# yanconglin/ICP-Flow

Measured on AMD Instinct MI355X. Metric: cluster-pair ICP registrations/sec, higher is better.
Workload: dtype f32

## Files before the change

icp_flow_amd/_lib.py:

```python
import contextlib
import ctypes
import os
import threading

import torch

_HERE = os.path.dirname(os.path.abspath(__file__))
LIB_PATH = os.environ.get("ICPFLOW_HIP_LIB") or os.path.join(_HERE, "libicpflow_hip.so")

STOP_REFERENCE = 0
STOP_PER_PAIR = 1

if not os.path.exists(LIB_PATH):
    raise ImportError(
        f"{LIB_PATH} not found: build it with `python icp_flow_amd/build.py` "
        "(hipcc --offload-arch=gfx950).  icp_flow_amd has no CPU fallback.")

_L = ctypes.CDLL(LIB_PATH)

_f = ctypes.c_float
_d = ctypes.c_double
_i = ctypes.c_int
_p = ctypes.c_void_p
_sz = ctypes.c_size_t
# ... 2 lines not shown
    "icpflow_version": (_i, []),
    "icpflow_last_error": (ctypes.c_char_p, []),
    "icpflow_workspace_bytes": (_sz, [_i, _i, _i, _i, _i]),
    "icpflow_hist_vote": (_i, [_p, _p, _i, _i, _i, _f, _f, _f, _f, _f, _f, _i, _i, _i, _p, _p]),
    "icpflow_hist_peaks": (_i, [_p, _i, _i, _i, _i, _i, _i, _p, _p, _p, _sz, _p]),
    "icpflow_nn_batch": (_i, [_p, _p, _i, _i, _i, _i, _i, _p, _p, _i, _p, _p, _p]),
    "icpflow_transform_points": (_i, [_p, _p, _i, _i, _p, _p]),
    "icpflow_count_valid": (_i, [_p, _i, _i, _p, _p]),
    "icpflow_build_info": (ctypes.c_char_p, []),
    "icpflow_estimate_init_pose": (_i, [_p, _p, _i, _i, _p, _i, _p, _i, _p, _i, _f, _p, _p, _sz, _p, _p]),
    "icpflow_icp": (_i, [_p, _p, _p, _i, _i, _d, _i, _d, _i, _p, _p, _p, _p, _p, _p, _sz, _p, _p]),
    "icpflow_apply_icp": (_i, [_p, _p, _p, _i, _i, _d, _i, _d, _i, _p, _p, _p, _sz, _p, _p]),
    "icpflow_hist_icp": (_i, [_p, _p, _i, _i, _p, _i, _p, _i, _p, _i, _f, _d, _i, _d, _i, _p, _p, _p, _sz, _p, _p]),
    "icpflow_hist_icp_many": (_i, [_i, _p, _p, _p, _i, _p, _i, _p, _i, _p, _i, _f, _d, _i, _d, _i, _p, _p, _p, _p, _p, _p]),
    "icpflow_match_eval": (_i, [_p, _p, _p, _i, _i, _d, _p, _p, _p, _p, _p, _p, _p, _sz, _p, _p]),
    "icpflow_hist_icp_eval": (_i, [_p, _p, _i, _i, _p, _i, _p, _i, _p, _i, _f, _d, _i, _d, _i, _p, _p, _p, _p, _p, _p, _p,
                                   _p, _p, _sz, _p, _p]),
    "icpflow_gather_pad": (_i, [_p, _p, _i, _i, _p, _p]),
    "icpflow_gather_segments": (_i, [_p, _p, _p, _p, _i, _i, _p, _p]),
    "icpflow_assoc_assign": (_i, [_p, _p, _p, _i, _p, _i, _i, _f, _f, _f, _f, _p, _i, _p, _p, _p, _p, _p]),
    "icpflow_assoc_collect": (_i, [_p, _p, _p, _p, _i, _p, _p, _p, _p, _i, _p, _p, _i, _i, _i, _p, _p, _p, _p]),
    "icpflow_register_stage": (_i, [_p, _p, _p, _p, _sz, _p, _p]),
    "icpflow_associate_frame": (_i, [_p, _p, _p, _p, _p, _f, _f, _f, _f, _p, _i, _p, _p, _p, _p, _i, _p, _p, _p, _sz, _p, _p]),
    "icpflow_register_stage_begin": (_i, [_p, _p, _p, _p, _sz, _p, _p, _p]),
    "icpflow_register_stage_finish": (_i, [_p, _p, _p, _p, _sz, _p, _p, _p]),
    "icpflow_associate_frame_begun": (_i, [_p, _p, _p, _p, _p, _f, _f, _f, _f, _p, _i, _p, _p, _p, _p, _i, _p, _p, _p, _sz, _p, _p, _p]),
    "icpflow_track_frame": (_i, [_p, _p, _i, _p, _p, _i, _p, _p, _p, _p, _p, _p, _p, _p, _p, _sz, _p, _p, _p]),
    "icpflow_selftest_randperm": (_i, [_p, ctypes.c_int64, _i, _p]),
    "icpflow_cluster_stats": (_i, [_p, _p, _p, _p, _p, _i, _p, _p, _p]),
    "icpflow_cluster_table_workspace_bytes": (_sz, [_i, _i]),
    "icpflow_cluster_table": (_i, [_p, _p, _i, _p, _p, _i, _p, _p, _sz, _p]),
    "icpflow_cluster_table_pair_workspace_bytes": (_sz, [_i, _i, _i]),
    "icpflow_cluster_table_pair": (_i, [_p, _p, _i, _p, _p, _p, _p, _p, _i, _p, _p, _p, _i, _p, _sz, _p]),
    "icpflow_flow_rigid": (_i, [_p, _p, _i, _p, _p, _i, _p, _p, _p, _sz, _p]),
    "icpflow_flow_rigid_rows": (_i, [_p, _p, _i, _p, _i, _p, _i, _p, _p, _p]),
    "icpflow_dbscan_workspace_bytes": (_sz, [_i]),
    "icpflow_dbscan": (_i, [_p, _i, _p, _i, _d, _i, _p, _p, _p, _p, _sz, _p]),
    "icpflow_hdbscan_mst_workspace_bytes": (_sz, [_i]),
    "icpflow_hdbscan_mst": (_i, [_p, _i, _p, _i, _i, _d, _p, _p, _p, _p, _p, _p, _p, _sz, _p]),
    "icpflow_hdbscan_labels": (_i, [_p, _p, _p, _i, _i, _p]),
    "icpflow_ego_default_params": (_i, [_p]),
    "icpflow_ego_state_bytes": (_sz, [_p]),
    "icpflow_ego_create": (_i, [_p, _p, _sz, _p, ctypes.POINTER(_p)]),
    "icpflow_ego_destroy": (_i, [_p]),
    "icpflow_ego_reset": (_i, [_p, _p]),
    "icpflow_ego_register_frame": (_i, [_p, _p, _i, _p, _p]),
    "icpflow_ego_poses": (_i, [_p, _p, _i, ctypes.POINTER(_i)]),
    "icpflow_ego_frame_info": (_i, [_p, _p]),
    "icpflow_ego_downsample": (_i, [_p, _p, _i, _p, _p, _p, _p]),
    "icpflow_ego_register_step": (_i, [_p, _p, _i, _p, _d, _p, _p]),
    "icpflow_ego_map_add": (_i, [_p, _p, _i, _p, _p]),
    "icpflow_ego_map_export": (_i, [_p, _p, _p, _p, _i, _p, _p]),
    "icpflow_selftest_vote_quotient": (_i, [_p, _i, _f, _f, _p, _p, _p]),
    "icpflow_selftest_kabsch": (_i, [_p, _p, _i, _i, _p, _p, _p, _p]),
    "icpflow_profile_create": (_i, [_i, ctypes.POINTER(_p)]),
    "icpflow_profile_collect": (_i, [_p, ctypes.POINTER(_d), ctypes.POINTER(_i)]),
    "icpflow_profile_destroy": (_i, [_p]),
}
for _name, (_res, _args) in SIGNATURES.items():
    _fn = getattr(_L, _name)
    _fn.restype = _res
    _fn.argtypes = _args

VERSION = int(_L.icpflow_version())
BUILD_INFO = _L.icpflow_build_info().decode()


def call(name, *args):
    rc = getattr(_L, name)(*args)
    if rc != 0:
        msg = _L.icpflow_last_error()
        raise RuntimeError(f"{name} failed (code {rc}): {msg.decode() if msg else ''}")


SEARCH_AUTO, SEARCH_SCAN, SEARCH_GRID, SEARCH_SWEEP = 0, 1, 2, 3
ARITH_FP64, ARITH_FP32_REFERENCE = 0, 1
OPT_FLAGS = {"no_sorted_vote": 1 << 0, "no_side_stream": 1 << 1, "no_eval_sweep": 1 << 2, "no_check_sweep": 1 << 3,
             "no_score_sweep": 1 << 4, "no_score_prune": 1 << 5, "no_teams": 1 << 6, "no_speculative": 1 << 7,
             "no_adaptive_windows": 1 << 8, "no_persistent": 1 << 9, "no_helpers": 1 << 10,
             "teams_half_gpu": 1 << 11, "no_shared_scans": 1 << 12,
             "no_stage_overlap": 1 << 13, "no_vote_list": 1 << 14, "no_check_reuse": 1 << 15, "no_score_prebound": 1 << 16,
             "two_launch": 1 << 17,
             "no_dir_keys": 1 << 18}


class Options(ctypes.Structure):
    _fields_ = [("struct_size", _sz), ("icp_search", _i), ("icp_arith", _i), ("flags", ctypes.c_uint),
                ("profile", _p), ("d_vote_bins_u32", _p), ("d_icp_init_R", _p), ("d_icp_init_T", _p),
                ("d_icp_history", _p), ("icp_allow_reflection", _i), ("icp_estimate_scale", _i),
                ("d_icp_scale", _p), ("d_icp_init_s", _p), ("d_pair_active", _p)]


class Tables(ctypes.Structure):
    _fields_ = [("d_points_src", _p), ("d_order_src", _p), ("d_table_src", _p), ("d_points_dst", _p), ("d_order_dst", _p),
                ("d_table_dst", _p), ("S", _i), ("D", _i), ("label_stride", _i)]


class Stage(ctypes.Structure):
    _fields_ = [("d_seg", _p), ("d_perm", _p), ("d_si", _p), ("d_di", _p), ("d_clouds", _p), ("d_result", _p), ("K", _i), ("N", _i)]


class Registration(ctypes.Structure):
    _fields_ = [("d_edges_x", _p), ("d_edges_y", _p), ("d_edges_z", _p), ("len_x", _i), ("len_y", _i), ("len_z", _i),
                ("decode_shift", _f), ("thres_dist", _d), ("relative_rmse_thr", _d), ("max_iterations", _i), ("stop_mode", _i)]


class Mt19937(ctypes.Structure):
    _fields_ = [("state", ctypes.c_uint32 * 624), ("index", ctypes.c_int32)]

    @staticmethod
    def from_torch(generator=None):
        raw = (generator if generator is not None else torch.default_generator).get_state().numpy()
        if raw.size < 24 + 8 * 624:
            raise RuntimeError("unexpected layout of torch.Generator.get_state()")
        left = int(raw[8:12].view("<i4")[0])
        nxt = int(raw[16:24].view("<u8")[0])
        mt = Mt19937()
        ctypes.memmove(mt.state, raw[24:24 + 8 * 624].view("<u8").astype("<u4").tobytes(), 4 * 624)
        mt.index = 624 if left == 1 else nxt
        return mt

    def to_torch(self, generator=None):
        import numpy as np
        g = generator if generator is not None else torch.default_generator
        raw = g.get_state().numpy().copy()
        raw[24:24 + 8 * 624] = np.frombuffer(bytes(self.state), dtype="<u4").astype("<u8").view(np.uint8)
        idx = int(self.index)
        raw[8:12] = np.array([1 if idx >= 624 else 625 - idx], "<i4").view(np.uint8)
        raw[16:24] = np.array([idx], "<u8").view(np.uint8)
        g.set_state(torch.from_numpy(raw))


class FrameParams(ctypes.Structure):
    _fields_ = [("struct_size", _sz), ("seed", ctypes.c_uint64), ("generator", _p), ("max_points", _i), ("min_cluster_size", _i),
                ("translation_frame", _f), ("thres_box", _f), ("thres_iou", _f), ("rot_limit_deg", _f), ("thres_error", _f),
                ("tight_padding", _i), ("superset_width", _i)]


class EgoParams(ctypes.Structure):
    _fields_ = [("struct_size", _sz), ("max_range", _d), ("min_range", _d), ("voxel_size", _d), ("min_motion_th", _d),
                ("initial_threshold", _d), ("convergence", _d), ("max_points_per_voxel", _i), ("max_iterations", _i),
                ("max_points", _i), ("map_capacity", _i)]

    @staticmethod
    def defaults(**over):
        p = EgoParams()
        call("icpflow_ego_default_params", ctypes.byref(p))
        for k, v in over.items():
            if not hasattr(p, k):
                raise TypeError(f"icpflow_ego_params_t has no field {k!r}")
            setattr(p, k, v)
        return p


class Profile:

    def __init__(self, capacity):
        self._h = _p()
        call("icpflow_profile_create", int(capacity), ctypes.byref(self._h))

    def collect(self):
        ms, n = _d(0.0), _i(0)
        call("icpflow_profile_collect", self._h, ctypes.byref(ms), ctypes.byref(n))
        return float(ms.value), int(n.value)

    def close(self):
        if self._h:
            _L.icpflow_profile_destroy(self._h)
            self._h = _p()

    __del__ = close


_tls = threading.local()


def _env_default_flags():
    f = 0
    for name, bit in OPT_FLAGS.items():
        if os.environ.get("ICPFLOW_" + name.upper(), "0") not in ("0", ""):
            f |= bit
    return f


_DEFAULT_FLAGS = _env_default_flags()


def _current():
    return getattr(_tls, "stack", None) or [dict(search=0, arith=0, flags=_DEFAULT_FLAGS, profile=None, vote_bins=None,
                                                 icp_init=None, icp_history=None, icp_allow_reflection=False,
                                                 icp_scale=None, pair_active=None)]


@contextlib.contextmanager
def options(search=None, arith=None, profile=None, vote_bins=None, icp_init=None, icp_history=None,
            icp_allow_reflection=None, icp_scale=None, pair_active=None, **switches):
    cur = dict(_current()[-1])
    cur.update(vote_bins=None, icp_init=None, icp_history=None, icp_scale=None, pair_active=None)
    if search is not None:
        cur["search"] = {"auto": 0, "scan": 1, "grid": 2, "sweep": 3}.get(search, search)
    if arith is not None:
        cur["arith"] = {"fp64": 0, "fp32_reference": 1}.get(arith, arith)
    if profile is not None:
        cur["profile"] = profile
    if vote_bins is not None:
        cur["vote_bins"] = vote_bins
    if icp_init is not None:
        cur["icp_init"] = icp_init
    if icp_history is not None:
        cur["icp_history"] = icp_history
    if icp_allow_reflection is not None:
        cur["icp_allow_reflection"] = bool(icp_allow_reflection)
    if icp_scale is not None:
        cur["icp_scale"] = icp_scale
    if pair_active is not None:
        cur["pair_active"] = pair_active
    for k, v in switches.items():
        cur["flags"] = (cur["flags"] | OPT_FLAGS[k]) if v else (cur["flags"] & ~OPT_FLAGS[k])
    stack = getattr(_tls, "stack", None)
    if stack is None:
        stack = _tls.stack = []
    stack.append(cur)
    try:
        yield
    finally:
        stack.pop()


def opt():
    cur = _current()[-1]
    if (cur["search"] == 0 and cur["arith"] == 0 and cur["flags"] == 0 and cur["profile"] is None
            and cur["vote_bins"] is None and cur["icp_init"] is None and cur["icp_history"] is None
            and not cur["icp_allow_reflection"] and cur["icp_scale"] is None and cur.get("pair_active") is None):
        return None
    dp = lambda t: ctypes.c_void_p(t.data_ptr()) if t is not None else None
    o = Options(int(os.environ.get("ICPFLOW_OPTIONS_SIZE", ctypes.sizeof(Options))), int(cur["search"]), int(cur["arith"]), int(cur["flags"]),
                cur["profile"]._h if cur["profile"] is not None else None, dp(cur["vote_bins"]),
                dp(cur["icp_init"][0] if cur["icp_init"] is not None else None),
                dp(cur["icp_init"][1] if cur["icp_init"] is not None else None), dp(cur["icp_history"]),
                1 if cur["icp_allow_reflection"] else 0, 1 if cur["icp_scale"] is not None else 0, dp(cur["icp_scale"]),
                dp(cur["icp_init"][2] if cur["icp_init"] is not None and len(cur["icp_init"]) > 2 else None),
                dp(cur.get("pair_active")))
    _tls.last = o
    return ctypes.cast(ctypes.pointer(o), _p)


def workspace_bytes(B, N, lens=(0, 0, 0)):
    return int(_L.icpflow_workspace_bytes(int(B), int(N), int(lens[0]), int(lens[1]), int(lens[2])))


def require_gpu(*tensors):
    for t in tensors:
        if t is None:
            continue
        if not isinstance(t, torch.Tensor) or not t.is_cuda:
            raise RuntimeError("icp_flow_amd: input must be a GPU (HIP) tensor -- there is no CPU path "
                               "(the reference refuses CPU tensors too, hist_cuda/cpp/hist.cpp:22)")


def cloud(t, name="cloud"):
    require_gpu(t)
    if t.dim() != 3 or t.shape[2] != 4:
        raise RuntimeError(f"{name}: expected shape [B,N,4] (x,y,z,flag), got {tuple(t.shape)}")
    if t.dtype != torch.float32:
        raise RuntimeError(f"{name}: expected float32, got {t.dtype}")
    return t.contiguous()


def ptr(t):
    return ctypes.c_void_p(t.data_ptr()) if t is not None else None


_raw_stream = getattr(torch._C, "_cuda_getCurrentRawStream", None)


def stream_handle(device):
    if _raw_stream is not None:
        idx = device.index if isinstance(device, torch.device) else None
        if idx is None:
            idx = torch.cuda.current_device()
        return int(_raw_stream(idx))
    return int(torch.cuda.current_stream(device).cuda_stream)


def stream(device):
    return ctypes.c_void_p(stream_handle(device))


_ws_cache = {}


def workspace(device, nbytes):
    key = (device.type, device.index, stream_handle(device))
    buf = _ws_cache.get(key)
    if buf is None or buf.numel() < nbytes:
        buf = torch.empty(max(int(nbytes), 1 << 20), dtype=torch.uint8, device=device)
        _ws_cache[key] = buf
    return buf


def workspaces(device, sizes):
# ... 20 lines not shown
```

icp_flow_amd/csrc/api.hip:

```cpp
#include <stdarg.h>
#include <stdio.h>
#include <stdlib.h>
#include <string.h>

#include "kernels.hpp"
#include "posefuse.hpp"
#include "kabsch.hpp"

using namespace icpflow;

namespace {

thread_local char g_err[512] = "";

int fail(int code, const char *fmt, ...)
{
    va_list ap;
    va_start(ap, fmt);
    vsnprintf(g_err, sizeof(g_err), fmt, ap);
    va_end(ap);
    return code;
}

int hipfail(hipError_t e, const char *what)
// ... 60 lines not shown
    int arith = ICPFLOW_ARITH_FP64;
    unsigned flags = 0u;
    LaunchProfile *profile = nullptr;
    uint32_t *voteBins = nullptr;
    const float *initR = nullptr, *initT = nullptr;
    float *history = nullptr;
    bool allowReflection = false;
    bool estimateScale = false;
    float *scaleOut = nullptr;
    const float *initS = nullptr;
    const uint8_t *pairActive = nullptr;
    bool on(unsigned offFlag) const { return (flags & offFlag) == 0u; }
    IcpOpts icp(float *scratch) const
    {
        IcpOpts o;
        o.fp32Scratch = scratch;
        o.ctrlCleared = true;
        o.arith = arith;
        o.teams = on(ICPFLOW_OPT_NO_TEAMS);
        o.speculative = on(ICPFLOW_OPT_NO_SPECULATIVE);
        o.adaptiveWindows = on(ICPFLOW_OPT_NO_ADAPTIVE_WINDOWS);
        o.persistent = on(ICPFLOW_OPT_NO_PERSISTENT);
        o.helpers = on(ICPFLOW_OPT_NO_HELPERS);
        o.teamsHalfGpu = (flags & ICPFLOW_OPT_TEAMS_HALF_GPU) != 0u;
        o.sharedScans = on(ICPFLOW_OPT_NO_SHARED_SCANS);
        o.twoLaunch = (flags & ICPFLOW_OPT_TWO_LAUNCH) != 0u;
        o.pairActive = pairActive;
        o.profile = profile;
        return o;
    }
};

#ifndef ICPFLOW_SCORE_SWEEP_MIN_N
#define ICPFLOW_SCORE_SWEEP_MIN_N 2048
#endif
constexpr int kScoreSweepMinN = ICPFLOW_SCORE_SWEEP_MIN_N;
constexpr int kMaxSortN = 16384;
inline bool eval_by_sweep(int B, int N, const Opts &o)
{
    if (N > kMaxSortN || !o.on(ICPFLOW_OPT_NO_EVAL_SWEEP)) return false;
    return N > kScoreSweepMinN || (N >= 1024 && (long long)B * N >= (1LL << 18));
}
#ifndef ICPFLOW_SCORE_SWEEP_MIN_N_SORTED
#define ICPFLOW_SCORE_SWEEP_MIN_N_SORTED 512
#endif
constexpr int kScoreSweepMinNSorted = ICPFLOW_SCORE_SWEEP_MIN_N_SORTED;
inline bool score_by_sweep(int N, bool sortedAnyway, const Opts &o)
{
    const int minN = (sortedAnyway && o.on(ICPFLOW_OPT_NO_SCORE_PRUNE)) ? kScoreSweepMinNSorted : kScoreSweepMinN;
    return N > minN && N <= kMaxSortN && o.on(ICPFLOW_OPT_NO_SCORE_SWEEP);
}
constexpr size_t kAlign = 256;
size_t up(size_t n) { return (n + kAlign - 1) / kAlign * kAlign; }

struct Workspace {
    int32_t *lenA = nullptr, *lenC = nullptr;
    uint8_t *swap = nullptr;
    uint32_t *bins = nullptr, *volA = nullptr, *volB = nullptr;
    float *peakVotes = nullptr;
    int64_t *peakIdx = nullptr;
    float *cand = nullptr;
    double *scoreAccum = nullptr;
    double *partial = nullptr;
    float *Tinit = nullptr, *M = nullptr;
    IcpState *state = nullptr;
    IcpCtrl *ctrl = nullptr;
    float *helpState = nullptr;
    double *helpOut = nullptr;
    GridScratch grid{};
    float *history = nullptr;
    float *zsortA = nullptr, *zsortC = nullptr;
    float *zckey = nullptr;
    int32_t *voteWork = nullptr;
    size_t voteWorkCap = 0;
    int32_t *pairTab = nullptr;
    int32_t *pairOrder = nullptr;
    float *pairBox = nullptr;
    float *voteKey = nullptr;
    int *zcidx = nullptr;
    IcpTeam team{};
    int32_t *icpSplit = nullptr;
    bool initSumValid = false;
    int *ticketScratch = nullptr;
    size_t accumBytes = 0;
    size_t bytes = 0;
    static bool shareScratch(int B, int N) { return N >= 2048 && (size_t)B * 12 * kSweepShareSlots * 256 * 4 <= ((size_t)64 << 20); }

    Workspace(void *base, int B, int N, size_t L)
    {
        size_t off = 0;
        auto take = [&](size_t n) {
            void *p = base ? (void *)((char *)base + off) : nullptr;
            off += up(n);
            return p;
        };
        const size_t b = (size_t)B;
        lenA = (int32_t *)take(b * 4);
        lenC = (int32_t *)take(b * 4);
        swap = (uint8_t *)take(b);
        bins = (uint32_t *)take(b * L * 4);
        volA = (uint32_t *)take(b * L * 4);
        volB = (uint32_t *)take(b * L * 4);
        peakVotes = (float *)take(b * kTopK * 4);
        peakIdx = (int64_t *)take(b * kTopK * 8);
        cand = (float *)take(b * kCand * 3 * 4);
        {
            size_t qb = (size_t)(scan_qblocks(N, B) > sweep_qblocks(N) ? scan_qblocks(N, B) : sweep_qblocks(N));
            if ((size_t)score_qblocks(N) > qb) qb = (size_t)score_qblocks(N);
            partial = (double *)take(b * 12 * qb * kPartial * 8);
            scoreAccum = (double *)take(b * 12 * 8);
            ticketScratch = (int *)take(256);
            if (shareScratch(B, N)) grid.shareCount = (int *)take(b * 12 * kSweepShareSlots * 4);
            accumBytes = up(b * 12 * 8) + up(256) + (shareScratch(B, N) ? up(b * 12 * kSweepShareSlots * 4) : 0);
        }
        Tinit = (float *)take(b * 16 * 4);
        M = (float *)take(b * 16 * 4);
        state = (IcpState *)take(b * sizeof(IcpState));
        ctrl = (IcpCtrl *)take(icp_ctrl_bytes(B));
        helpState = (float *)take(b * 32 * 4);
        helpOut = (double *)take((size_t)kHelpMaxWG * kHelpOutStride * 8);
        grid.H = grid_buckets(N);
        grid.origin = (float *)take(b * 4 * 4);
        grid.start = (int32_t *)take(b * ((size_t)grid.H + 1) * 4);
        grid.cursor = (int32_t *)take(b * (size_t)grid.H * 4);
        grid.pts = (float *)take(b * (size_t)N * 16);
        grid.sortX = (float *)take(b * (size_t)N * 16);
        grid.sortYsoa = (float *)take(b * 3 * (size_t)((N + 15) / 16 * 16) * 4 + 256);
        grid.sortXsoa = (float *)take(b * 3 * (size_t)((N + 15) / 16 * 16) * 4 + 256);
        zsortA = (float *)take(b * (size_t)N * 16);
        zsortC = (float *)take(b * (size_t)N * 16);
        voteKey = (float *)take(b * 8 * 4);
        voteWorkCap = vote_work_capacity(B, N);
        if (voteWorkCap != 0) { voteWork = (int32_t *)take(voteWorkCap * 4); pairOrder = (int32_t *)take(b * 4); }
        if (N > kChunkSortMinN) {
            const size_t cs = b * 2 * (size_t)chunk_sort_length(N) * 4;
            grid.ckey = (float *)take(cs);
            grid.cidx = (int *)take(cs);
            zckey = (float *)take(cs);
            zcidx = (int *)take(cs);
            pairBox = (float *)take(b * kPairBoxStride * 4);
        }
        grid.axis = (int32_t *)take(b * 4);
        grid.scoreList = (int *)take(b * 12 * 4);
        if (N <= kMaxSortN) {
            grid.occHdr = (float *)take(b * 2 * 8 * 4);
            grid.occBits = (uint32_t *)take(b * 2 * (size_t)kOccRings * kOccWords * 4);
        }
        if (shareScratch(B, N)) {
            grid.shareBest = (float *)take(b * 12 * kSweepShareSlots * 256 * 4);
            if (B <= 32767 && N <= 255 * 256) pairTab = (int32_t *)take(b * 4 * 4);
        }
        history = (float *)take(b * (size_t)kHistIters * kHistStride * 4);
        team.maxWG = 1024;
        team.wgPair = (int32_t *)take((size_t)team.maxWG * 4);
        team.wgRank = (int32_t *)take((size_t)team.maxWG * 4);
        team.teamSize = (int32_t *)take(b * 4);
        team.next = (int32_t *)take(b * 4);
        team.arrived = (unsigned int *)take(b * 4);
        team.mom = (double *)take((b < 256 ? b : 256) * 2 * (size_t)kMaxTeam * kTeamStride * 8);
        icpSplit = (int32_t *)take((b + 64) * 4);
        bytes = off;
    }
};

const GridScratch *search_scratch(Workspace &w, int N, const Opts &o)
{
    int mode = o.search;
    if (o.arith == ICPFLOW_ARITH_FP32_REFERENCE) mode = 1;
    if (mode == 0) mode = (N >= 64 && N <= kMaxSortN) ? 3 : 1;
    if (mode == 3 && N > kMaxSortN) mode = 1;
    if (mode == 1) return nullptr;
    w.grid.mode = mode;
    w.grid.dirKeys = o.on(ICPFLOW_OPT_NO_DIR_KEYS) ? 1 : 0;
    return &w.grid;
}

int parse_options(const char *fn, const icpflow_options_t *opt, Opts &o)
{
    if (opt == nullptr) return 0;
    if (opt->struct_size != sizeof(icpflow_options_t))
        return fail(ICPFLOW_E_ARG, "%s: options struct_size %zu, this library expects %zu", fn, opt->struct_size,
                    sizeof(icpflow_options_t));
    if (opt->icp_search < 0 || opt->icp_search > 3)
        return fail(ICPFLOW_E_ARG, "%s: options.icp_search must be 0..3 (got %d)", fn, opt->icp_search);
    if (opt->icp_arith != ICPFLOW_ARITH_FP64 && opt->icp_arith != ICPFLOW_ARITH_FP32_REFERENCE)
        return fail(ICPFLOW_E_ARG, "%s: options.icp_arith must be 0 or 1 (got %d)", fn, opt->icp_arith);
    if (opt->flags >> 19) return fail(ICPFLOW_E_ARG, "%s: unknown option flags 0x%x", fn, opt->flags);
    o.search = opt->icp_search;
    o.arith = opt->icp_arith;
    o.flags = opt->flags;
    o.profile = reinterpret_cast<LaunchProfile *>(opt->profile);
    o.voteBins = opt->d_vote_bins_u32;
    if ((opt->d_icp_init_R == nullptr) != (opt->d_icp_init_T == nullptr))
        return fail(ICPFLOW_E_ARG, "%s: options.d_icp_init_R and d_icp_init_T come together", fn);
    o.initR = opt->d_icp_init_R;
    o.initT = opt->d_icp_init_T;
    o.history = opt->d_icp_history;
    o.allowReflection = opt->icp_allow_reflection != 0;
    o.estimateScale = opt->icp_estimate_scale != 0;
    o.scaleOut = opt->d_icp_scale;
    o.initS = opt->d_icp_init_s;
    o.pairActive = opt->d_pair_active;
    if (o.initS != nullptr && o.initR == nullptr)
        return fail(ICPFLOW_E_ARG, "%s: options.d_icp_init_s comes with d_icp_init_R / d_icp_init_T", fn);
    return 0;
}

int check_pair_active(const char *fn, const Opts &o, bool fused, int maxIter, int stopMode)
{
    if (o.pairActive == nullptr) return 0;
    if (!fused) return fail(ICPFLOW_E_ARG, "%s: options.d_pair_active is honoured by icpflow_hist_icp / icpflow_hist_icp_eval only", fn);
    if (stopMode != ICPFLOW_STOP_REFERENCE || maxIter < 2 || maxIter > kHistIters || !o.on(ICPFLOW_OPT_NO_SPECULATIVE) ||
        o.arith != ICPFLOW_ARITH_FP64)
        return fail(ICPFLOW_E_ARG, "%s: options.d_pair_active needs the single-launch reference stop (2 <= max_iterations <= %d, "
                                   "fp64 arithmetic, speculation on)", fn, kHistIters);
    return 0;
}

int check_arith(const char *fn, const Opts &o, int maxIter, int stopMode)
{
    if (o.arith != ICPFLOW_ARITH_FP32_REFERENCE) return 0;
    if (stopMode != ICPFLOW_STOP_REFERENCE)
        return fail(ICPFLOW_E_ARG, "%s: ICPFLOW_ARITH_FP32_REFERENCE implements the reference's batch-global stop only", fn);
    if (maxIter > kHistIters)
        return fail(ICPFLOW_E_LIMIT, "%s: ICPFLOW_ARITH_FP32_REFERENCE keeps a per-iteration history: max_iterations <= %d",
                    fn, kHistIters);
    return 0;
}

int check_ws(void *ws, size_t have, size_t need)
{
    if (ws == nullptr || have < need)
        return fail(ICPFLOW_E_WORKSPACE, "workspace too small: have %zu bytes, need %zu", have, need);
    if (((uintptr_t)ws & 15) != 0) return fail(ICPFLOW_E_WORKSPACE, "workspace must be 16-byte aligned");
    return 0;
}

int check_batch(const char *fn, int B, int N)
{
    if (B <= 0 || N <= 0) return fail(ICPFLOW_E_ARG, "%s: B (%d) and N (%d) must be positive", fn, B, N);
    if ((long long)B * N > (1ll << 30)) return fail(ICPFLOW_E_LIMIT, "%s: B*N exceeds 2^30 rows", fn);
    return 0;
}

int check_hist_dims(const char *fn, int lx, int ly, int lz)
{
    if (lx <= 0 || ly <= 0 || lz <= 0)
        return fail(ICPFLOW_E_ARG, "%s: histogram lengths must be positive (%d,%d,%d)", fn, lx, ly, lz);
    if ((long long)lx * ly * lz > (1ll << 28)) return fail(ICPFLOW_E_LIMIT, "%s: histogram too large", fn);
    return 0;
}

struct SideStream {
    hipStream_t stream = nullptr;
    hipEvent_t fork = nullptr, join = nullptr;
    int device = -1;
    bool ok = false;
    void destroy()
    {
        if (stream) (void)hipStreamDestroy(stream);
        if (fork) (void)hipEventDestroy(fork);
        if (join) (void)hipEventDestroy(join);
        stream = nullptr; fork = join = nullptr; ok = false;
    }
    void create()
    {
        ok = hipGetDevice(&device) == hipSuccess &&
             hipStreamCreateWithFlags(&stream, hipStreamNonBlocking) == hipSuccess &&
             hipEventCreateWithFlags(&fork, hipEventDisableTiming) == hipSuccess &&
             hipEventCreateWithFlags(&join, hipEventDisableTiming) == hipSuccess;
    }
};

SideStream &side_stream(hipStream_t caller)
{
    constexpr int kSlots = 6;
    struct Slot { SideStream s; hipStream_t caller = nullptr; bool used = false; };
    static thread_local Slot slots[kSlots];
    static thread_local int next = 0;
    static thread_local SideStream none;
    int dev = -1;
    if (hipGetDevice(&dev) != hipSuccess) { none.ok = false; return none; }
    for (int k = 0; k < kSlots; ++k)
        if (slots[k].used && slots[k].caller == caller && slots[k].s.device == dev) return slots[k].s;
    Slot &sl = slots[next];
    next = (next + 1) % kSlots;
    if (!sl.used || sl.s.device != dev) {
        sl.s.destroy();
        sl.s = SideStream{};
        sl.s.create();
    }
    sl.used = true;
    sl.caller = caller;
    return sl.s;
}

struct JoinGuard {
    hipStream_t s = nullptr;
    hipEvent_t join = nullptr;
    ~JoinGuard() { if (join != nullptr) (void)hipStreamWaitEvent(s, join, 0); }
    void joined() { join = nullptr; }
};

int run_icp_and_select(const float *src, const float *dst, Workspace &w, const uint8_t *swap,
                       const float *init, int B, int N, double thres, int maxIter, double relThr,
                       int stopMode, int invertSwapped, float *Tout, int32_t *iters, const Opts &o, hipStream_t s,
                       bool teamPlanned = false, int part = 0, int32_t *pending = nullptr, bool initSumValid = false)
{
    const GridScratch *search = search_scratch(w, N, o);
    const bool sweepCheck = search != nullptr && search->mode == 3 && o.on(ICPFLOW_OPT_NO_CHECK_SWEEP);
    bool historyPending = false;
    IcpOpts io = o.icp(w.grid.sortX);
    io.help = icp_help_carve(w.ctrl, B, w.helpState, w.helpOut);
    io.splitScratch = w.icpSplit;
    io.teamPlanned = teamPlanned;
    if (sweepCheck && o.arith == ICPFLOW_ARITH_FP64) io.historyPending = &historyPending;
    const bool splittable = sweepCheck && o.arith == ICPFLOW_ARITH_FP64 && stopMode == ICPFLOW_STOP_REFERENCE && w.history != nullptr &&
                            o.on(ICPFLOW_OPT_NO_SPECULATIVE) && maxIter > 1 && maxIter <= kHistIters;
    if (part == 1) {
        *pending = 0;
        if (!splittable) return 0;
        if (icp_teams_wanted(&w.team, io, search, B, N, maxIter, stopMode, w.history)) return 0;
        io.pairActive = nullptr;
    }
    if (part == 2 && pending != nullptr && *pending != 0) {
        historyPending = true;
        if (o.pairActive != nullptr) ICPFLOW_TRY(launch_icp_retally(w.ctrl, w.history, o.pairActive, B, maxIter, relThr, s));
    } else {
        ICPFLOW_TRY(launch_icp(src, dst, w.lenA, w.lenC, swap, init, B, N, thres, maxIter, relThr, stopMode,
                               w.state, w.ctrl, search, w.history, &w.team, io, s));
        if (part == 1) {
            if (!historyPending) return fail(ICPFLOW_E_ARG, "icpflow_register_stage_begin: the ICP launch kept no history");
            *pending = 1;
            return 0;
        }
    }
    if (sweepCheck) {
        PoseSource ps{w.state, w.ctrl, historyPending ? w.history : nullptr, init, B, maxIter};
        const double *initSum = (initSumValid && search->presorted && o.on(ICPFLOW_OPT_NO_CHECK_REUSE)) ? w.scoreAccum : nullptr;
        ICPFLOW_TRY(launch_sweep_check(search, src, dst, w.lenA, w.lenC, swap, B, N, init, nullptr, w.partial, s, &ps, o.pairActive,
                                       initSum));
        ICPFLOW_TRY(launch_select(w.partial, sweep_qblocks(N), w.lenA, w.lenC, swap, init, nullptr, B, invertSwapped,
                                  Tout, s, &ps, iters, initSum, o.pairActive));
        return 0;
    }
    ICPFLOW_TRY(launch_compose(w.state, init, B, w.M, s, w.ctrl, iters));
    {
        ICPFLOW_TRY(launch_scan_check(src, dst, w.lenA, w.lenC, swap, B, N, init, w.M, w.partial, s));
        ICPFLOW_TRY(launch_select(w.partial, scan_qblocks(N, B), w.lenA, w.lenC, swap, init, w.M, B,
                                  invertSwapped, Tout, s));
    }
    return 0;
}

int run_init_pose(const float *src, const float *dst, Workspace &w, const uint8_t *swap, int B,
                  int N, const float *ex, int lx, const float *ey, int ly, const float *ez, int lz,
                  float shift, float *Tout, const Opts &o, hipStream_t s, hipEvent_t joinBefore = nullptr,
                  const PairCountFuse *countFuse = nullptr, bool sideBusy = false)
{
    const int lens[3] = {lx, ly, lz};
    if (N <= kMaxSortN && o.on(ICPFLOW_OPT_NO_SORTED_VOTE)) {
        bool planned = false;
        ICPFLOW_TRY(launch_hist_vote_sorted(dst, src, w.lenC, w.lenA, B, N, lens, ex, ey, ez, swap, w.zsortC,
                                            w.zsortA, w.bins, w.zckey, w.zcidx, w.voteKey, s, countFuse, sideBusy,
                                            w.grid.pairBox, o.on(ICPFLOW_OPT_NO_VOTE_LIST) ? w.voteWork : nullptr, w.voteWorkCap,
                                            w.pairOrder, &planned));
        if (planned) w.grid.pairOrder = w.pairOrder;
    } else
        ICPFLOW_TRY(launch_hist_vote(dst, src, B, N, N, nullptr, nullptr, lens, ex, ey, ez, swap, w.bins, s));
    if (o.voteBins != nullptr)
        ICPFLOW_TRY(hipMemcpyAsync(o.voteBins, w.bins, (size_t)B * lx * ly * lz * sizeof(uint32_t),
                                   hipMemcpyDeviceToDevice, s));
    if (w.pairTab != nullptr && B <= 700 && N <= kMaxSortN && o.on(ICPFLOW_OPT_NO_SORTED_VOTE)) {
        ICPFLOW_TRY(launch_sweep_pair_table(w.lenA, w.lenC, swap, w.grid.pairOrder, B, N, w.pairTab, s));
        w.grid.pairTab = w.pairTab;
    }
    PeakDecode dec;
    dec.ex = ex; dec.ey = ey; dec.ez = ez; dec.shift = shift; dec.cand = w.cand;
    ICPFLOW_TRY(launch_hist_peaks_u32(w.bins, B, lx, ly, lz, kTopK, kNmsKernel, w.volA, w.volB,
                                      w.peakVotes, w.peakIdx, s, dec));
    if (score_by_sweep(N, joinBefore != nullptr || w.grid.presorted, o)) {
        if (joinBefore != nullptr) {
            ICPFLOW_TRY(hipStreamWaitEvent(s, joinBefore, 0));
        } else if (!w.grid.presorted) {
            ICPFLOW_TRY(launch_sort_clouds_soa(src, dst, w.lenA, w.lenC, swap, B, N, &w.grid, s));
            w.grid.presorted = 1;
            if (o.on(ICPFLOW_OPT_NO_SCORE_PRUNE) && o.on(ICPFLOW_OPT_NO_SCORE_PREBOUND)) {
                ICPFLOW_TRY(launch_occupancy(&w.grid, B, N, s));
                w.grid.occReady = 1;
            }
        }
        if (o.on(ICPFLOW_OPT_NO_SCORE_PRUNE))
            ICPFLOW_TRY(launch_sweep_score_pruned(&w.grid, w.lenA, w.lenC, swap, B, N, w.cand, w.partial, w.scoreAccum, s));
        else
            ICPFLOW_TRY(launch_sweep_score(&w.grid, w.lenA, w.lenC, swap, B, N, w.cand, w.partial, s));
        ICPFLOW_TRY(launch_score_pick(w.partial, sweep_qblocks(N), w.lenA, w.lenC, swap, w.cand, B, Tout, s, w.scoreAccum));
        w.initSumValid = true;
    } else if (o.on(ICPFLOW_OPT_NO_SCORE_PRUNE)) {
        ICPFLOW_TRY(launch_scan_score_pruned(src, dst, w.lenA, w.lenC, swap, B, N, w.cand, w.partial, w.scoreAccum, s, true));
        ICPFLOW_TRY(launch_score_pick(w.partial, score_qblocks(N), w.lenA, w.lenC, swap, w.cand, B, Tout, s));
    } else {
        ICPFLOW_TRY(launch_scan_score(src, dst, w.lenA, w.lenC, swap, B, N, w.cand, w.partial, s));
        ICPFLOW_TRY(launch_score_pick(w.partial, scan_qblocks(N, B), w.lenA, w.lenC, swap, w.cand, B, Tout, s));
    }
    return 0;
}

}

extern "C" {

int icpflow_version(void) { return ICPFLOW_VERSION; }

#ifndef ICPFLOW_SOURCE_HASH
#define ICPFLOW_SOURCE_HASH "unknown"
#endif
static const char g_build_info[] = "ICPFLOW_SOURCE_HASH=" ICPFLOW_SOURCE_HASH;
const char *icpflow_build_info(void) { return g_build_info + sizeof("ICPFLOW_SOURCE_HASH=") - 1; }

const char *icpflow_last_error(void) { return g_err; }

size_t icpflow_workspace_bytes(int B, int N, int Lx, int Ly, int Lz)
{
    if (B <= 0 || N <= 0) return 0;
    const size_t L = (size_t)(Lx > 0 ? Lx : 0) * (size_t)(Ly > 0 ? Ly : 0) * (size_t)(Lz > 0 ? Lz : 0);
    return Workspace(nullptr, B, N, L).bytes;
}

int icpflow_profile_create(int capacity, icpflow_profile_t **out)
{
    if (out == nullptr) return fail(ICPFLOW_E_ARG, "icpflow_profile_create: null pointer");
    if (capacity < 0 || capacity > (1 << 20)) return fail(ICPFLOW_E_ARG, "icpflow_profile_create: bad capacity %d", capacity);
    hipError_t e = hipSuccess;
    LaunchProfile *p = profile_create(capacity, &e);
    if (p == nullptr) return hipfail(e, "icpflow_profile_create");
    *out = reinterpret_cast<icpflow_profile_t *>(p);
    return 0;
}

int icpflow_profile_collect(icpflow_profile_t *profile, double *total_ms, int *launches)
{
    if (profile == nullptr) return fail(ICPFLOW_E_ARG, "icpflow_profile_collect: null recorder");
    ICPFLOW_TRY(profile_collect(reinterpret_cast<LaunchProfile *>(profile), total_ms, launches));
    return 0;
}

int icpflow_profile_destroy(icpflow_profile_t *profile)
{
    profile_destroy(reinterpret_cast<LaunchProfile *>(profile));
    return 0;
}

int icpflow_selftest_vote_quotient(const float *d_a, int n, float min_v, float max_v, float *d_fast,
                                   float *d_ieee, icpflow_stream_t stream)
{
    if (!d_a || !d_fast || !d_ieee) return fail(ICPFLOW_E_ARG, "icpflow_selftest_vote_quotient: null pointer");
    if (n <= 0) return fail(ICPFLOW_E_ARG, "icpflow_selftest_vote_quotient: n must be positive");
    ICPFLOW_TRY(launch_vote_quotient_probe(d_a, n, min_v, max_v, d_fast, d_ieee, (hipStream_t)stream));
    return 0;
}

int icpflow_selftest_kabsch(const double *d_H, const double *d_gsum, int n, int mode, double *d_R, double *d_lam,
                            int32_t *d_path, icpflow_stream_t stream)
{
    if (!d_H || !d_R || !d_lam || !d_path || (mode != 2 && !d_gsum))
        return fail(ICPFLOW_E_ARG, "icpflow_selftest_kabsch: null pointer");
    if (n <= 0 || n > (1 << 24)) return fail(ICPFLOW_E_ARG, "icpflow_selftest_kabsch: bad n %d", n);
    if (mode < 0 || mode > 2) return fail(ICPFLOW_E_ARG, "icpflow_selftest_kabsch: bad mode %d", mode);
    ICPFLOW_TRY(launch_kabsch_probe(d_H, d_gsum, n, mode, d_R, d_lam, d_path, (hipStream_t)stream));
    return 0;
}

int icpflow_hist_vote(const float *d_X, const float *d_Y, int B, int NX, int NY, float min_x,
                      float min_y, float min_z, float max_x, float max_y, float max_z, int len_x,
                      int len_y, int len_z, float *d_bins, icpflow_stream_t stream)
{
    if (!d_X || !d_Y || !d_bins) return fail(ICPFLOW_E_ARG, "icpflow_hist_vote: null pointer");
    if (int r = check_batch("icpflow_hist_vote", B, NX)) return r;
    if (int r = check_batch("icpflow_hist_vote", B, NY)) return r;
    if (int r = check_hist_dims("icpflow_hist_vote", len_x, len_y, len_z)) return r;
// ... 286 lines not shown
        return fail(ICPFLOW_E_WORKSPACE, "icpflow_cluster_table: workspace too small (%zu bytes, need %zu)", ws_bytes,
                    icpflow_cluster_table_workspace_bytes(M, Lmax));
    return 0;
}

size_t icpflow_cluster_table_pair_workspace_bytes(int MA, int MB, int Lmax)
{
    if (MA <= 0 || MB <= 0 || Lmax <= 0 || (long long)MA + MB > 0x7fffffffll) return 0;
    size_t bytes = 0;
    if (cluster_table_pair_workspace_bytes(MA, MB, Lmax, &bytes) != hipSuccess) return 0;
    return bytes;
}

int icpflow_cluster_table_pair(const float *d_points_a, const float *d_labels_a, int MA, int64_t *d_order_a, double *d_table_a,
                               int32_t *d_num_a, const float *d_points_b, const float *d_labels_b, int MB,
                               int64_t *d_order_b, double *d_table_b, int32_t *d_num_b, int Lmax, void *d_ws, size_t ws_bytes,
                               icpflow_stream_t stream)
{
    if (!d_points_a || !d_labels_a || !d_order_a || !d_table_a || !d_num_a || !d_points_b || !d_labels_b || !d_order_b ||
        !d_table_b || !d_num_b)
        return fail(ICPFLOW_E_ARG, "icpflow_cluster_table_pair: null pointer");
    if (MA <= 0 || MB <= 0) return fail(ICPFLOW_E_ARG, "icpflow_cluster_table_pair: MA, MB must be positive (got %d, %d)", MA, MB);
    if ((long long)MA + MB > 0x7fffffffll)
        return fail(ICPFLOW_E_LIMIT, "icpflow_cluster_table_pair: MA + MB must stay below 2^31 (got %d + %d)", MA, MB);
    if (Lmax <= 0 || Lmax > 4096) return fail(ICPFLOW_E_LIMIT, "icpflow_cluster_table_pair: 1 <= Lmax <= 4096 (got %d)", Lmax);
    if (!d_ws) return fail(ICPFLOW_E_WORKSPACE, "icpflow_cluster_table_pair: workspace is NULL");
    bool tooSmall = false;
    ICPFLOW_TRY(launch_cluster_table_pair(d_points_a, d_labels_a, MA, d_order_a, d_table_a, d_num_a, d_points_b, d_labels_b, MB,
                                          d_order_b, d_table_b, d_num_b, Lmax, d_ws, ws_bytes, &tooSmall, (hipStream_t)stream));
    if (tooSmall)
        return fail(ICPFLOW_E_WORKSPACE, "icpflow_cluster_table_pair: workspace too small (%zu bytes, need %zu)", ws_bytes,
                    icpflow_cluster_table_pair_workspace_bytes(MA, MB, Lmax));
    return 0;
}

int icpflow_flow_rigid_rows(const float *d_points, const float *d_labels, int N, const float *d_pair_rows, int pair_stride,
                            const float *d_T, int P, const float *d_pose, float *d_flow, icpflow_stream_t stream)
{
    if (!d_points || !d_labels || !d_pose || !d_flow) return fail(ICPFLOW_E_ARG, "icpflow_flow_rigid: null pointer");
    if (N <= 0) return fail(ICPFLOW_E_ARG, "icpflow_flow_rigid: N must be positive");
    if (P < 0 || P > (1 << 24)) return fail(ICPFLOW_E_LIMIT, "icpflow_flow_rigid: 0 <= P <= 2^24 pairs (got %d)", P);
    if (P > 0 && (!d_pair_rows || !d_T)) return fail(ICPFLOW_E_ARG, "icpflow_flow_rigid: null pair arrays");
    if (pair_stride < 1 || pair_stride > 1024)
        return fail(ICPFLOW_E_ARG, "icpflow_flow_rigid: pair_stride must be in 1 ... 1024 floats (got %d)", pair_stride);
    ICPFLOW_TRY(launch_flow_rigid(d_points, d_labels, N, d_pair_rows, pair_stride, d_T, P, d_pose, d_flow, (hipStream_t)stream));
    return 0;
}

int icpflow_flow_rigid(const float *d_points, const float *d_labels, int N, const float *d_pair_labels,
                       const float *d_T, int P, const float *d_pose, float *d_flow, void *d_ws, size_t ws_bytes,
                       icpflow_stream_t stream)
{
    (void)d_ws;
    (void)ws_bytes;
    return icpflow_flow_rigid_rows(d_points, d_labels, N, d_pair_labels, 1, d_T, P, d_pose, d_flow, stream);
}

int icpflow_count_valid(const float *d_pts, int B, int N, int32_t *d_len, icpflow_stream_t stream)
{
    if (!d_pts || !d_len) return fail(ICPFLOW_E_ARG, "icpflow_count_valid: null pointer");
    if (int r = check_batch("icpflow_count_valid", B, N)) return r;
    launch_count_valid(d_pts, B, N, d_len, (hipStream_t)stream);
    ICPFLOW_TRY(hipGetLastError());
    return 0;
}

int icpflow_estimate_init_pose(const float *d_src, const float *d_dst, int B, int N,
                               const float *d_edges_x, int len_x, const float *d_edges_y, int len_y,
                               const float *d_edges_z, int len_z, float decode_shift, float *d_T_out,
                               void *d_ws, size_t ws_bytes, icpflow_stream_t stream, const icpflow_options_t *opt)
{
    Opts o;
    if (int r = parse_options("icpflow_estimate_init_pose", opt, o)) return r;
    if (int r = check_pair_active("icpflow_estimate_init_pose", o, false, 0, 0)) return r;
    if (!d_src || !d_dst || !d_edges_x || !d_edges_y || !d_edges_z || !d_T_out)
        return fail(ICPFLOW_E_ARG, "icpflow_estimate_init_pose: null pointer");
    if (int r = check_batch("icpflow_estimate_init_pose", B, N)) return r;
    if (int r = check_hist_dims("icpflow_estimate_init_pose", len_x, len_y, len_z)) return r;
    const size_t L = (size_t)len_x * len_y * len_z;
    if (L < (size_t)kTopK) return fail(ICPFLOW_E_ARG, "icpflow_estimate_init_pose: fewer than 5 bins");
    Workspace w(d_ws, B, N, L);
    if (int r = check_ws(d_ws, ws_bytes, w.bytes)) return r;
    hipStream_t s = (hipStream_t)stream;
    launch_count_pair(d_src, d_dst, B, N, w.lenA, w.lenC, nullptr, s, w.scoreAccum, (size_t)B * 12 * sizeof(double));
    return run_init_pose(d_src, d_dst, w, nullptr, B, N, d_edges_x, len_x, d_edges_y, len_y, d_edges_z,
                         len_z, decode_shift, d_T_out, o, s);
}

int icpflow_icp(const float *d_X, const float *d_Y, const float *d_pre_pose, int B, int N, double thres,
                int max_iterations, double relative_rmse_thr, int stop_mode, float *d_R, float *d_T,
                float *d_rmse, int32_t *d_iters, int32_t *d_converged, void *d_ws, size_t ws_bytes,
                icpflow_stream_t stream, const icpflow_options_t *opt)
{
    Opts o;
    if (int r = parse_options("icpflow_icp", opt, o)) return r;
    if (int r = check_pair_active("icpflow_icp", o, false, 0, 0)) return r;
    if (int r = check_arith("icpflow_icp", o, max_iterations, stop_mode)) return r;
    if (!d_X || !d_Y) return fail(ICPFLOW_E_ARG, "icpflow_icp: null pointer");
    if (int r = check_batch("icpflow_icp", B, N)) return r;
    if (max_iterations <= 0 || max_iterations > kMaxIterCap)
        return fail(ICPFLOW_E_ARG, "icpflow_icp: max_iterations must be in 1..%d (got %d)", kMaxIterCap, max_iterations);
    if (stop_mode != ICPFLOW_STOP_REFERENCE && stop_mode != ICPFLOW_STOP_PER_PAIR)
        return fail(ICPFLOW_E_ARG, "icpflow_icp: unknown stop_mode %d", stop_mode);
    Workspace w(d_ws, B, N, 0);
    if (int r = check_ws(d_ws, ws_bytes, w.bytes)) return r;
    hipStream_t s = (hipStream_t)stream;
    IcpOpts io = o.icp(w.grid.sortX);
    io.help = icp_help_carve(w.ctrl, B, w.helpState, w.helpOut);
    io.splitScratch = w.icpSplit;
    io.initR = o.initR;
    io.initT = o.initT;
    io.allowReflection = o.allowReflection;
    io.estimateScale = o.estimateScale;
    io.initS = o.initS;
    if ((o.allowReflection || o.estimateScale) && o.arith != ICPFLOW_ARITH_FP64)
        return fail(ICPFLOW_E_ARG, "icpflow_icp: allow_reflection / estimate_scale are not built for ICPFLOW_ARITH_FP32_REFERENCE");
    if (o.history != nullptr &&
        !(stop_mode == ICPFLOW_STOP_REFERENCE && max_iterations > 1 && max_iterations <= kHistIters &&
          o.arith == ICPFLOW_ARITH_FP64 && io.speculative))
        return fail(ICPFLOW_E_ARG, "icpflow_icp: options.d_icp_history needs the single-launch reference stop mode "
                                   "(2 <= max_iterations <= %d, fp64 arithmetic)", kHistIters);
    if (o.initR != nullptr && o.arith != ICPFLOW_ARITH_FP64)
        return fail(ICPFLOW_E_ARG, "icpflow_icp: an initial transform is not built for ICPFLOW_ARITH_FP32_REFERENCE");
    Opts os = o;
    if ((o.estimateScale || o.initS != nullptr) && o.search == 0 && N < 64) os.search = 3;
    const GridScratch *search = search_scratch(w, N, os);
    if ((o.estimateScale || o.initS != nullptr) && (search == nullptr || search->mode != 3))
        return fail(ICPFLOW_E_ARG, "icpflow_icp: estimate_scale / an initial transform with a scale need the sorted-sweep "
                                   "search (the default up to N = %d)", kMaxSortN);
    launch_count_pair(d_X, d_Y, B, N, w.lenA, w.lenC, nullptr, s, w.ctrl, icp_ctrl_bytes(B));
    ICPFLOW_TRY(launch_icp(d_X, d_Y, w.lenA, w.lenC, nullptr, d_pre_pose, B, N, thres, max_iterations,
                           relative_rmse_thr, stop_mode, w.state, w.ctrl, search, w.history, &w.team,
                           io, s));
    if (o.history != nullptr)
        ICPFLOW_TRY(hipMemcpyAsync(o.history, w.history, (size_t)max_iterations * B * kHistStride * sizeof(float),
                                   hipMemcpyDeviceToDevice, s));
    ICPFLOW_TRY(launch_icp_export(w.state, w.ctrl, B, stop_mode, d_R, d_T, d_rmse, d_iters, d_converged, s, o.scaleOut));
    return 0;
}

int icpflow_apply_icp(const float *d_src, const float *d_dst, const float *d_init, int B, int N,
                      double thres_dist, int max_iterations, double relative_rmse_thr, int stop_mode,
                      float *d_T_out, int32_t *d_iters, void *d_ws, size_t ws_bytes,
                      icpflow_stream_t stream, const icpflow_options_t *opt)
{
    Opts o;
    if (int r = parse_options("icpflow_apply_icp", opt, o)) return r;
    if (int r = check_arith("icpflow_apply_icp", o, max_iterations, stop_mode)) return r;
    if (int r = check_pair_active("icpflow_apply_icp", o, false, max_iterations, stop_mode)) return r;
    if (!d_src || !d_dst || !d_init || !d_T_out) return fail(ICPFLOW_E_ARG, "icpflow_apply_icp: null pointer");
    if (int r = check_batch("icpflow_apply_icp", B, N)) return r;
    if (max_iterations <= 0 || max_iterations > kMaxIterCap)
        return fail(ICPFLOW_E_ARG, "icpflow_apply_icp: max_iterations must be in 1..%d", kMaxIterCap);
    if (stop_mode != ICPFLOW_STOP_REFERENCE && stop_mode != ICPFLOW_STOP_PER_PAIR)
        return fail(ICPFLOW_E_ARG, "icpflow_apply_icp: unknown stop_mode %d", stop_mode);
    Workspace w(d_ws, B, N, 0);
    if (int r = check_ws(d_ws, ws_bytes, w.bytes)) return r;
    hipStream_t s = (hipStream_t)stream;
    launch_count_pair(d_src, d_dst, B, N, w.lenA, w.lenC, nullptr, s, w.ctrl, icp_ctrl_bytes(B));
    ICPFLOW_TRY(hipMemcpyAsync(w.Tinit, d_init, (size_t)B * 16 * sizeof(float), hipMemcpyDeviceToDevice, s));
    return run_icp_and_select(d_src, d_dst, w, nullptr, w.Tinit, B, N, thres_dist, max_iterations,
                              relative_rmse_thr, stop_mode, 0, d_T_out, d_iters, o, s);
}

static int hist_icp_core(const float *d_src, const float *d_dst, int B, int N, const float *d_edges_x, int len_x,
                         const float *d_edges_y, int len_y, const float *d_edges_z, int len_z, float decode_shift,
                         double thres_dist, int max_iterations, double relative_rmse_thr, int stop_mode,
                         float *d_T_out, int32_t *d_iters, Workspace &w, const Opts &o, hipStream_t s,
                         int phase = 0, int32_t *carry = nullptr)
{
    if (phase == 2) {
        w.grid.presorted = carry[0];
        w.grid.shareCountClean = 1;
        int32_t pending = carry[2];
        return run_icp_and_select(d_src, d_dst, w, w.swap, w.Tinit, B, N, thres_dist, max_iterations,
                                  relative_rmse_thr, stop_mode, 1, d_T_out, d_iters, o, s, carry[1] != 0, 2, &pending, carry[3] != 0);
    }
    const bool countInSort = N <= kMaxSortN && N <= kChunkSortMinN && o.on(ICPFLOW_OPT_NO_SORTED_VOTE);
    if (!countInSort) {
        launch_count_pair(d_src, d_dst, B, N, w.lenA, w.lenC, w.swap, s, w.ctrl, icp_ctrl_bytes(B), w.scoreAccum,
                          w.accumBytes, w.pairBox);
        w.grid.pairBox = w.pairBox;
    }
    hipEvent_t join = nullptr;
    bool teamPlanned = false;
    JoinGuard guard;
    const GridScratch *search = search_scratch(w, N, o);
    SideStream *side = nullptr;
    if (search != nullptr && search->mode == 3 && N >= 64 && o.on(ICPFLOW_OPT_NO_SIDE_STREAM)) {
        side = &side_stream(s);
        if (!side->ok) side = nullptr;
    }
    if (side != nullptr) {
        ICPFLOW_TRY(hipEventRecord(side->fork, s));
        ICPFLOW_TRY(hipStreamWaitEvent(side->stream, side->fork, 0));
        hipError_t se = launch_sort_clouds_soa(d_src, d_dst, w.lenA, w.lenC, w.swap, B, N, &w.grid, side->stream,
                                               countInSort ? 2 : 0);
        if (se == hipSuccess && score_by_sweep(N, true, o) && o.on(ICPFLOW_OPT_NO_SCORE_PRUNE) && o.on(ICPFLOW_OPT_NO_SCORE_PREBOUND)) {
            se = launch_occupancy(&w.grid, B, N, side->stream);
            if (se == hipSuccess) w.grid.occReady = 1;
        }
        if (se == hipSuccess && !countInSort && phase != 1 &&
            icp_teams_wanted(&w.team, o.icp(w.grid.sortX), search, B, N, max_iterations, stop_mode, w.history)) {
            launch_icp_team_plan(&w.team, w.lenA, w.lenC, w.swap, B, N, o.icp(w.grid.sortX), side->stream);
            teamPlanned = true;
        }
        const hipError_t je = hipEventRecord(side->join, side->stream);
        if (je == hipSuccess) { guard.s = s; guard.join = side->join; }
        ICPFLOW_TRY(se);
        ICPFLOW_TRY(je);
        w.grid.presorted = 1;
        join = side->join;
    }
    PairCountFuse fuse{};
    if (countInSort) {
        fuse.swapOut = w.swap;
        fuse.zero0 = w.ctrl; fuse.bytes0 = icp_ctrl_bytes(B);
        fuse.zero1 = w.scoreAccum; fuse.bytes1 = w.accumBytes;
    }
    w.grid.shareCountClean = 1;
    w.grid.sweepTicket = w.ticketScratch;
    const bool sweepScore = score_by_sweep(N, join != nullptr, o);
    if (int r = run_init_pose(d_src, d_dst, w, w.swap, B, N, d_edges_x, len_x, d_edges_y, len_y, d_edges_z,
                              len_z, decode_shift, w.Tinit, o, s, sweepScore ? join : nullptr,
                              countInSort ? &fuse : nullptr, join != nullptr))
        return r;
    if (join != nullptr && !sweepScore) ICPFLOW_TRY(hipStreamWaitEvent(s, join, 0));
    guard.joined();
    if (phase == 1) {
        carry[0] = w.grid.presorted;
        carry[1] = teamPlanned ? 1 : 0;
        carry[3] = w.initSumValid ? 1 : 0;
        return run_icp_and_select(d_src, d_dst, w, w.swap, w.Tinit, B, N, thres_dist, max_iterations, relative_rmse_thr,
                                  stop_mode, 1, d_T_out, d_iters, o, s, teamPlanned, 1, &carry[2]);
    }
    return run_icp_and_select(d_src, d_dst, w, w.swap, w.Tinit, B, N, thres_dist, max_iterations,
                              relative_rmse_thr, stop_mode, 1, d_T_out, d_iters, o, s, teamPlanned, 0, nullptr, w.initSumValid);
}

int icpflow_hist_icp(const float *d_src, const float *d_dst, int B, int N, const float *d_edges_x,
                     int len_x, const float *d_edges_y, int len_y, const float *d_edges_z, int len_z,
                     float decode_shift, double thres_dist, int max_iterations, double relative_rmse_thr,
                     int stop_mode, float *d_T_out, int32_t *d_iters, void *d_ws, size_t ws_bytes,
                     icpflow_stream_t stream, const icpflow_options_t *opt)
{
    Opts o;
    if (int r = parse_options("icpflow_hist_icp", opt, o)) return r;
    if (int r = check_arith("icpflow_hist_icp", o, max_iterations, stop_mode)) return r;
    if (int r = check_pair_active("icpflow_hist_icp", o, true, max_iterations, stop_mode)) return r;
    if (!d_src || !d_dst || !d_edges_x || !d_edges_y || !d_edges_z || !d_T_out)
        return fail(ICPFLOW_E_ARG, "icpflow_hist_icp: null pointer");
    if (int r = check_batch("icpflow_hist_icp", B, N)) return r;
    if (int r = check_hist_dims("icpflow_hist_icp", len_x, len_y, len_z)) return r;
    if (max_iterations <= 0 || max_iterations > kMaxIterCap)
        return fail(ICPFLOW_E_ARG, "icpflow_hist_icp: max_iterations must be in 1..%d", kMaxIterCap);
    if (stop_mode != ICPFLOW_STOP_REFERENCE && stop_mode != ICPFLOW_STOP_PER_PAIR)
        return fail(ICPFLOW_E_ARG, "icpflow_hist_icp: unknown stop_mode %d", stop_mode);
    const size_t L = (size_t)len_x * len_y * len_z;
    if (L < (size_t)kTopK) return fail(ICPFLOW_E_ARG, "icpflow_hist_icp: fewer than 5 bins");
    Workspace w(d_ws, B, N, L);
    if (int r = check_ws(d_ws, ws_bytes, w.bytes)) return r;
    return hist_icp_core(d_src, d_dst, B, N, d_edges_x, len_x, d_edges_y, len_y, d_edges_z, len_z, decode_shift,
                         thres_dist, max_iterations, relative_rmse_thr, stop_mode, d_T_out, d_iters, w, o,
                         (hipStream_t)stream);
}

int icpflow_hist_icp_many(int K, const float *const *d_src, const float *const *d_dst, const int *B, int N,
                          const float *d_edges_x, int len_x, const float *d_edges_y, int len_y,
                          const float *d_edges_z, int len_z, float decode_shift, double thres_dist,
                          int max_iterations, double relative_rmse_thr, int stop_mode, float *const *d_T_out,
                          int32_t *const *d_iters, void *const *d_ws, const size_t *ws_bytes,
                          icpflow_stream_t stream, const icpflow_options_t *opt)
{
    if (K <= 0 || K > 64) return fail(ICPFLOW_E_ARG, "icpflow_hist_icp_many: K must be in 1..64 (got %d)", K);
    if (!d_src || !d_dst || !B || !d_T_out || !d_iters || !d_ws || !ws_bytes)
        return fail(ICPFLOW_E_ARG, "icpflow_hist_icp_many: null pointer");
    for (int k = 0; k < K; ++k)
        for (int j = 0; j < k; ++j)
            if (d_ws[k] == d_ws[j]) return fail(ICPFLOW_E_WORKSPACE, "icpflow_hist_icp_many: batches %d and %d share a workspace", j, k);
    hipStream_t s = (hipStream_t)stream;
    constexpr int kWorkers = 4;
    struct Pool {
        hipStream_t w[kWorkers] = {nullptr, nullptr, nullptr, nullptr};
        hipEvent_t fork = nullptr, join[kWorkers] = {nullptr, nullptr, nullptr, nullptr};
        int device = -1;
        bool ok = false;
    };
    static thread_local Pool pool;
    int dev = -1;
    ICPFLOW_TRY(hipGetDevice(&dev));
    if (!pool.ok || pool.device != dev) {
        pool = Pool{};
        pool.device = dev;
        ICPFLOW_TRY(hipEventCreateWithFlags(&pool.fork, hipEventDisableTiming));
        for (int k = 0; k < kWorkers; ++k) {
            ICPFLOW_TRY(hipStreamCreateWithFlags(&pool.w[k], hipStreamNonBlocking));
            ICPFLOW_TRY(hipEventCreateWithFlags(&pool.join[k], hipEventDisableTiming));
        }
        pool.ok = true;
    }
    const int used = K < kWorkers ? K : kWorkers;
    ICPFLOW_TRY(hipEventRecord(pool.fork, s));
    for (int k = 0; k < used; ++k) ICPFLOW_TRY(hipStreamWaitEvent(pool.w[k], pool.fork, 0));
    int rc = 0;
    for (int k = 0; k < K && rc == 0; ++k)
        rc = icpflow_hist_icp(d_src[k], d_dst[k], B[k], N, d_edges_x, len_x, d_edges_y, len_y, d_edges_z, len_z, decode_shift,
                              thres_dist, max_iterations, relative_rmse_thr, stop_mode, d_T_out[k], d_iters[k], d_ws[k],
                              ws_bytes[k], pool.w[k % kWorkers], opt);
    for (int k = 0; k < used; ++k) {
        const hipError_t e1 = hipEventRecord(pool.join[k], pool.w[k]);
        const hipError_t e2 = e1 == hipSuccess ? hipStreamWaitEvent(s, pool.join[k], 0) : e1;
        if (rc == 0 && e2 != hipSuccess) rc = hipfail(e2, "icpflow_hist_icp_many: join");
    }
    return rc;
}
// ... 126 lines not shown
```

icp_flow_amd/csrc/kernels.hpp:

```cpp
#pragma once
#include <hip/hip_runtime.h>
#include <atomic>
#include <stddef.h>
#include <stdint.h>

#include "../../include/icpflow_hip.h"

namespace icpflow {

constexpr int ICPFLOW_STOP_REFERENCE_ = ICPFLOW_STOP_REFERENCE;
constexpr int ICPFLOW_STOP_PER_PAIR_ = ICPFLOW_STOP_PER_PAIR;

constexpr int kPartial = 8;
constexpr int kMaxIterCap = 1024;
constexpr int kCand = 6;
constexpr int kTopK = 5;
constexpr int kNmsKernel = 11;

struct IcpState {
    float R[9];
    float T[3];
    float rmse;
    int active;
    int iters;
// ... 41 lines not shown
struct IcpTeam {
    int32_t *wgPair;
    int32_t *wgRank;
    int32_t *teamSize;
    int32_t *next;
    unsigned int *arrived;
    double *mom;
    int maxWG;
};

inline size_t icp_ctrl_bytes(int B)
{
    return sizeof(IcpCtrl) + (size_t)B * sizeof(HelpPair) + 2 * (size_t)kHelpMaxWG * sizeof(int);
}
inline IcpHelp icp_help_carve(IcpCtrl *ctrl, int B, float *state, double *out)
{
    IcpHelp h;
    h.pair = reinterpret_cast<HelpPair *>(ctrl + 1);
    h.tag = reinterpret_cast<int *>(h.pair + B);
    h.owner = h.tag + kHelpMaxWG;
    h.state = state;
    h.out = out;
    return h;
}

constexpr int kHistIters = 128;
constexpr int kHistStride = 16;

void launch_count_valid(const float *pts, int B, int N, int32_t *len, hipStream_t s);
void launch_count_pair(const float *A, const float *C, int B, int N, int32_t *lenA, int32_t *lenC, uint8_t *swap,
                       hipStream_t s, void *zero0 = nullptr, size_t bytes0 = 0, void *zero1 = nullptr, size_t bytes1 = 0,
                       float *boxes = nullptr);
hipError_t launch_hist_vote(const float *X, const float *Y, int B, int NX, int NY,
                            const float mins[3], const float maxs[3], const int lens[3],
                            const float *ex, const float *ey, const float *ez,
                            const uint8_t *swap, uint32_t *bins_u32, hipStream_t s);
struct PairCountFuse {
    uint8_t *swapOut;
    void *zero0; size_t bytes0;
    void *zero1; size_t bytes1;
};
hipError_t launch_hist_vote_sorted(const float *X, const float *Y, int32_t *nX, int32_t *nY,
                                   int B, int N, const int lens[3], const float *ex, const float *ey,
                                   const float *ez, const uint8_t *swap, float *sortX, float *sortY,
                                   uint32_t *bins_u32, float *ckey, int *cidx, float *keyRec, hipStream_t s,
                                   const PairCountFuse *fuse = nullptr, bool sideBusy = false, const float *boxes = nullptr,
                                   int32_t *work = nullptr, size_t workCap = 0, int32_t *orderOut = nullptr, bool *planned = nullptr);
size_t vote_work_capacity(int B, int N);
constexpr int kChunkSortMinN = 4096;
constexpr int kPairBoxStride = 24;
int chunk_sort_length(int N);
hipError_t launch_zsort_chunked(const float *P, const float *Q, const int32_t *nP, const int32_t *nQ, int B, int N,
                                float *outP, float *outQ, uint32_t *bins, int L, float *ckey, int *cidx,
                                const float *ez, int len_z, float *keyRec, hipStream_t s, const float *boxes = nullptr);
hipError_t launch_sort_clouds_chunked(const float *X, const float *Y, const int32_t *lenX, const int32_t *lenY,
                                      const uint8_t *swap, const float *prePose, int B, int N, int32_t *axisOut,
                                      float *Xs, float *Ys, float *Ysoa, float *Xsoa, float *ckey, int *cidx,
                                      hipStream_t s, const float *boxes = nullptr, int dirKeys = 0);
hipError_t launch_u32_to_f32(const uint32_t *in, float *out, size_t n, hipStream_t s);
hipError_t launch_hist_peaks_f32(const float *bins, int B, int Lx, int Ly, int Lz, int k,
                                 int kernel_size, uint32_t *wsA, uint32_t *wsB, float *votes,
                                 int64_t *idx, hipStream_t s);
struct PeakDecode {
    const float *ex = nullptr, *ey = nullptr, *ez = nullptr;
    float shift = 0.f;
    float *cand = nullptr;
};
hipError_t launch_hist_peaks_u32(const uint32_t *bins, int B, int Lx, int Ly, int Lz, int k,
                                 int kernel_size, uint32_t *wsA, uint32_t *wsB, float *votes,
                                 int64_t *idx, hipStream_t s, PeakDecode dec = PeakDecode{});

struct GridScratch;
hipError_t launch_sweep_pair_table(const int32_t *lenA, const int32_t *lenC, const uint8_t *swap, const int32_t *pairOrder,
                                   int B, int N, int32_t *tab, hipStream_t s);
int scan_qblocks(int maxRows, int batch);
int sweep_qblocks(int maxRows);
hipError_t launch_sweep_eval(const GridScratch *grid, const int32_t *len1, const int32_t *len2, int B, int N,
                             const float *pose, float thres, float *srcT, double *partial, hipStream_t s, const uint8_t *swap = nullptr,
                             const uint8_t *active = nullptr);
struct PoseSource;
hipError_t launch_sweep_check(const GridScratch *grid, const float *X, const float *Y, const int32_t *lenA,
                              const int32_t *lenC, const uint8_t *swap, int B, int N, const float *poseInit,
                              const float *poseFinal, double *partial, hipStream_t s, const PoseSource *fused = nullptr,
                              const uint8_t *active = nullptr, const double *initSum = nullptr);
hipError_t launch_occupancy(const GridScratch *grid, int B, int N, hipStream_t s);
hipError_t launch_sweep_score(const GridScratch *grid, const int32_t *lenA, const int32_t *lenC, const uint8_t *swap,
                              int B, int N, const float *cand, double *partial, hipStream_t s);
hipError_t launch_sweep_score_pruned(const GridScratch *grid, const int32_t *lenA, const int32_t *lenC,
                                     const uint8_t *swap, int B, int N, const float *cand, double *partial,
                                     double *accum, hipStream_t s);
hipError_t launch_scan_score(const float *A, const float *C, const int32_t *lenA, const int32_t *lenC,
                             const uint8_t *swap, int B, int N, const float *cand, double *partial,
                             hipStream_t s);
int score_qblocks(int maxRows);
hipError_t launch_scan_score_pruned(const float *A, const float *C, const int32_t *lenA, const int32_t *lenC,
                                    const uint8_t *swap, int B, int N, const float *cand, double *partial,
                                    double *accum, hipStream_t s, bool accumCleared = false);
hipError_t launch_scan_check(const float *A, const float *C, const int32_t *lenA, const int32_t *lenC,
                             const uint8_t *swap, int B, int N, const float *poseInit,
                             const float *poseFinal, double *partial, hipStream_t s);
hipError_t launch_scan_eval(const float *A, const float *C, const int32_t *lenA, const int32_t *lenC,
                            int B, int N, const float *pose, float thres, double *partial, hipStream_t s);
hipError_t launch_scan_nn(const float *Qp, const float *Tp, int B, int NQ, int NT, int strideQ,
                          int strideT, const int32_t *lenQ, const int32_t *lenT, int sqrt_dist,
                          int64_t *idx, float *dist, hipStream_t s);

constexpr int kOccWords = 1024;
#ifndef ICPFLOW_OCC_RINGS
#define ICPFLOW_OCC_RINGS 3
#endif
constexpr int kOccRings = ICPFLOW_OCC_RINGS;
constexpr int kSweepShareSlots = 16;
struct GridScratch {
    int mode;
    int H;
    float *origin;
    int32_t *start;
    int32_t *cursor;
    float *pts;
    float *sortX;
    float *sortYsoa;
    float *sortXsoa;
    int32_t *axis;
    int dirKeys;
    float *ckey;
    int *cidx;
    const float *pairBox;
    const int32_t *pairTab;
    const int32_t *pairOrder;
    float *shareBest;
    int *shareCount;
    int shareCountClean;
    float *occHdr;
    uint32_t *occBits;
    int occReady;
    int *sweepTicket;
    int *scoreList;
    int presorted;
};
int grid_buckets(int N);
struct LaunchProfile;
struct IcpOpts {
    int arith = 0;
    bool teams = true;
    bool speculative = true;
    bool adaptiveWindows = true;
    bool persistent = true;
    bool helpers = true;
    IcpHelp help{};
    const float *initR = nullptr;
    const float *initT = nullptr;
    bool allowReflection = false;
    bool estimateScale = false;
    const float *initS = nullptr;
    LaunchProfile *profile = nullptr;
    bool ctrlCleared = false;
    bool *historyPending = nullptr;
    float *fp32Scratch = nullptr;
    bool teamPlanned = false;
    const uint8_t *pairActive = nullptr;
    bool teamsHalfGpu = false;
    bool sharedScans = true;
    bool twoLaunch = false;
    int32_t *splitScratch = nullptr;
};
bool icp_teams_wanted(const IcpTeam *team, const IcpOpts &opts, const GridScratch *grid, int B, int N, int maxIter,
                      int stopMode, const float *history);
int icp_team_workgroups(const IcpOpts &opts);
void launch_icp_team_plan(const IcpTeam *team, const int32_t *lenX, const int32_t *lenY, const uint8_t *swap, int B, int N,
                          const IcpOpts &opts, hipStream_t s);
hipError_t launch_icp_fp32ref(const float *X, const float *Y, const int32_t *lenX, const int32_t *lenY,
                              const uint8_t *swap, const float *prePose, int B, int N, double thres, int maxIter,
                              double relThr, IcpState *state, IcpCtrl *ctrl, float *history, float *nnScratch,
                              hipStream_t s);
hipError_t launch_icp(const float *X, const float *Y, const int32_t *lenX, const int32_t *lenY,
                      const uint8_t *swap, const float *prePose, int B, int N, double thres,
                      int maxIter, double relThr, int stopMode, IcpState *state, IcpCtrl *ctrl,
                      const GridScratch *grid, float *history, const IcpTeam *team, const IcpOpts &opts,
                      hipStream_t s);
hipError_t launch_sort_clouds_soa(const float *X, const float *Y, const int32_t *lenX, const int32_t *lenY,
                                  const uint8_t *swap, int B, int N, const GridScratch *grid, hipStream_t s, int selfCount = 0);
LaunchProfile *profile_create(int capacity, hipError_t *err);
void profile_destroy(LaunchProfile *p);
hipError_t profile_collect(LaunchProfile *p, double *total_ms, int *launches);
int device_cus();
void ensure_dynamic_lds(const void *func, int bytes, std::atomic<unsigned long long> *doneMask);
hipError_t launch_icp_export(IcpState *state, IcpCtrl *ctrl, int B, int stopMode, float *R,
                             float *T, float *rmse, int32_t *iters, int32_t *converged, hipStream_t s,
                             float *scale = nullptr);
hipError_t launch_icp_retally(IcpCtrl *ctrl, const float *history, const uint8_t *active, int B, int maxIter, double relThr,
                              hipStream_t s);
hipError_t launch_icp_resolve_history(IcpState *state, IcpCtrl *ctrl, const float *history, int B, int maxIter,
                                      hipStream_t s);

hipError_t launch_score_pick(const double *partial, int qblocks, const int32_t *lenA,
                             const int32_t *lenC, const uint8_t *swap, const float *cand, int B,
                             float *Tinit, hipStream_t s, double *initSum = nullptr);
hipError_t launch_compose(const IcpState *state, const float *init, int B, float *M, hipStream_t s,
                          const IcpCtrl *ctrl = nullptr, int32_t *iters = nullptr);
hipError_t launch_select(const double *partial, int qblocks, const int32_t *lenA, const int32_t *lenC,
                         const uint8_t *swap, const float *init, const float *M, int B, int invertSwapped,
                         float *out, hipStream_t s, const PoseSource *fused = nullptr, int32_t *iters = nullptr,
                         const double *initSum = nullptr, const uint8_t *active = nullptr);
hipError_t launch_eval_epilogue(const double *partial, int qblocks, const int32_t *len1,
                                const int32_t *len2, const float *T, int B, float *errors,
                                float *inliers, float *ratios, float *ious, float *translations,
                                float *rotations, hipStream_t s);
hipError_t launch_vote_quotient_probe(const float *a, int n, float mn, float mx, float *fast, float *ieee,
                                      hipStream_t s);
hipError_t launch_kabsch_probe(const double *H, const double *gsum, int n, int mode, double *R, double *lam, int32_t *path,
                               hipStream_t s);
hipError_t launch_gather_pad(const float *points, const int32_t *rows, int B, int N, float *out, hipStream_t s);
hipError_t launch_gather_segments(const float *points, const int64_t *order, const int64_t *seg, const int32_t *perm,
                                  int B, int N, float *out, hipStream_t s);
hipError_t launch_cluster_stats(const float *points, const int64_t *order, const int64_t *start,
                                const int64_t *count, const float *labels, int L, float *mean, float *extent,
                                hipStream_t s);
hipError_t launch_flow_rigid(const float *points, const float *labels, int N, const float *pairRows, int pairStride,
                             const float *T, int P, const float *pose, float *flow, hipStream_t s);
hipError_t launch_transform_points(const float *xyz, const float *pose, int B, int N, float *out,
// ... 33 lines not shown
```

icp_flow_amd/csrc/nn.hip:

```cpp
#include "scan.hpp"
#include "sortdir.hpp"
#include "kernels.hpp"
#include "posefuse.hpp"

namespace icpflow {

enum ScanMode : int { MODE_SCORE = 0, MODE_CHECK = 1, MODE_EVAL = 2, MODE_NN = 3 };

struct ScanParams {
    const float *A;
    const float *C;
    const int32_t *lenA;
    const int32_t *lenC;
    const uint8_t *swap;
    int N;
    int NT;
    int strideQ, strideT;
    int njobs;
    int qblocks;
    const float *cand;
    int subBegin, subCount, prune;
    double *accum;
    int split;
    const float *poseA;
    const float *poseB;
    float thres;
    double *partial;
    int64_t *idx;
    float *dist;
    int sqrt_dist;
};

template <int Q, int MODE>
__global__ __launch_bounds__(kScanBlock) void nn_scan_kernel(ScanParams p)
{
    __shared__ ScanTile tileMem;
    ScanTile *tile = &tileMem;
    __shared__ double red[(kScanBlock / kWave) * kPartial];

    const int lin = blockIdx.x;
    int job = (lin / (8 * p.qblocks)) * 8 + (lin & 7);
    int qb = (lin >> 3) % p.qblocks;
    if (MODE == MODE_SCORE && p.prune) {
        const int padded = (p.njobs + 7) & ~7;
        qb = lin / padded;
        job = lin % padded;
    }
    if (job >= p.njobs) return;

    int b, sub;
    if (MODE == MODE_SCORE) {
        b = job / p.subCount;
        sub = p.subBegin + job % p.subCount;
        job = b * 12 + sub;
    }
    else if (MODE == MODE_NN) { b = job; sub = 0; }
    else { b = job >> 1; sub = job & 1; }

    CloudView qc, tc;
    PointXf qxf, txf;
    qxf.kind = XF_NONE; txf.kind = XF_NONE;
    qxf.a = affine_identity(); txf.a = qxf.a;

    if (MODE == MODE_NN) {
        qc.base = p.A + (size_t)b * p.N * p.strideQ; qc.stride = p.strideQ;
        qc.n = p.lenA ? p.lenA[b] : p.N;
        tc.base = p.C + (size_t)b * p.NT * p.strideT; tc.stride = p.strideT;
        tc.n = p.lenC ? p.lenC[b] : p.NT;
    } else {
        const bool sw = p.swap != nullptr && p.swap[b] != 0;
        CloudView a, c;
        a.base = (sw ? p.C : p.A) + (size_t)b * p.N * 4; a.stride = 4; a.n = (sw ? p.lenC : p.lenA)[b];
        c.base = (sw ? p.A : p.C) + (size_t)b * p.N * 4; c.stride = 4; c.n = (sw ? p.lenA : p.lenC)[b];
        PointXf axf;
        axf.a = affine_identity();
        if (MODE == MODE_SCORE) {
            const int k = sub >> 1;
            axf.kind = XF_TRANSLATE;
            const float *t = p.cand + ((size_t)b * 6 + k) * 3;
            axf.a.t[0] = t[0]; axf.a.t[1] = t[1]; axf.a.t[2] = t[2];
        } else if (MODE == MODE_CHECK) {
            axf.kind = XF_AFFINE;
            axf.a = affine_from_pose((sub == 0 ? p.poseA : p.poseB) + (size_t)b * 16);
        } else {
            axf.kind = XF_AFFINE;
            axf.a = affine_from_pose(p.poseA + (size_t)b * 16);
// ... 119 lines not shown
    double v[kPartial];
#pragma unroll
    for (int k = 0; k < kPartial; ++k) v[k] = 0.0;
#pragma unroll
    for (int q = 0; q < Q; ++q) {
        if (!live[q]) continue;
        const float d = sqrtf(acc.best[q]);
        v[0] += (double)d;
        if (MODE == MODE_EVAL) {
            v[1] += (d < p.thres) ? 1.0 : 0.0;
            if (sub == 0) {
                v[2] += (double)qx[q]; v[3] += (double)qy[q]; v[4] += (double)qz[q];
                v[5] += (double)ox[q]; v[6] += (double)oy[q]; v[7] += (double)oz[q];
            }
        }
    }
    block_sum<kPartial, double>(v, red);
    if (threadIdx.x == 0) {
        double *o = p.partial + ((size_t)job * p.qblocks + qb) * kPartial;
#pragma unroll
        for (int k = 0; k < kPartial; ++k) o[k] = v[k];
        if (MODE == MODE_SCORE && p.accum != nullptr) atomicAdd(p.accum + job, v[0]);
    }
}

static int scan_queries_per_lane(int maxRows, int batch)
{
    if (maxRows <= 512) return 1;
    if (maxRows <= 1024 || batch <= 128) return 2;
    return 4;
}

template <int MODE>
static hipError_t launch_scan(ScanParams p, int maxRows, int batch, hipStream_t s)
{
    const int Q = scan_queries_per_lane(maxRows, batch);
    p.qblocks = (maxRows + kScanBlock * Q - 1) / (kScanBlock * Q);
    const int groups = (p.njobs + 7) / 8;
    const dim3 grid((unsigned)(groups * 8 * p.qblocks));
    if (Q == 1) hipLaunchKernelGGL((nn_scan_kernel<1, MODE>), grid, dim3(kScanBlock), 0, s, p);
    else if (Q == 2) hipLaunchKernelGGL((nn_scan_kernel<2, MODE>), grid, dim3(kScanBlock), 0, s, p);
    else hipLaunchKernelGGL((nn_scan_kernel<4, MODE>), grid, dim3(kScanBlock), 0, s, p);
    return hipGetLastError();
}

int scan_qblocks(int maxRows, int batch)
{
    const int Q = scan_queries_per_lane(maxRows, batch);
    return (maxRows + kScanBlock * Q - 1) / (kScanBlock * Q);
}

struct SweepParams {
    const float *Asoa;
    const float *Csoa;
    const int32_t *lenA, *lenC;
    const uint8_t *swap;
    const int32_t *axis;
    const float *cand;
    const float4 *sortX;
    const float *X, *Y;
    const float *poseA, *poseB;
    PoseSource fused;
    int rawSorted;
    const float *srcT;
    float thres;
    int N, NP16, njobs, qblocks;
    float r0;
    double *partial;
    int subBegin, subCount, prune;
    double *accum;
    float *shareBest;
    int *shareCount;
    int shareClean;
    int shareWindows;
    const int32_t *pairTab;
    const int32_t *pairOrder;
    const uint8_t *active;
    const double *initSum;
    const float *occHdr;
    const uint32_t *occBits;
    int listMode;
    int *list, *listCount;
    int boundBoth;
};

#ifdef ICPFLOW_OCC_STATS
__device__ unsigned long long g_occStats[12];
__device__ unsigned int g_occPair[1024];
#endif
constexpr int kSweepBlock = 256;
#ifndef ICPFLOW_SWEEP_SHARE_MIN_TARGETS
#define ICPFLOW_SWEEP_SHARE_MIN_TARGETS 512
#endif
constexpr int kSweepShareMinTargets = ICPFLOW_SWEEP_SHARE_MIN_TARGETS;
#ifndef ICPFLOW_SWEEP_FULLSCAN_MIN_TARGETS
#define ICPFLOW_SWEEP_FULLSCAN_MIN_TARGETS 2048
#endif
constexpr int kSweepFullScanMinTargets = ICPFLOW_SWEEP_FULLSCAN_MIN_TARGETS;
constexpr int kSweepShares = 8;
#ifndef ICPFLOW_SWEEP_FULLSCAN_QBLOCKS
#define ICPFLOW_SWEEP_FULLSCAN_QBLOCKS 2
#endif
constexpr int kSweepFullQb = ICPFLOW_SWEEP_FULLSCAN_QBLOCKS;
#ifndef ICPFLOW_SWEEP_FULLSCAN_MIN_NT
#define ICPFLOW_SWEEP_FULLSCAN_MIN_NT 512
#endif
constexpr int kSweepFullScanMinNt = ICPFLOW_SWEEP_FULLSCAN_MIN_NT;
static_assert(kSweepFullQb * kSweepShares <= kSweepShareSlots, "GridScratch.shareBest holds kSweepShareSlots records of 256 minima per job");
constexpr int kSweepStage = 4096;
enum SweepMode : int { SWEEP_SCORE = 0, SWEEP_CHECK = 1, SWEEP_EVAL = 2 };

#ifdef ICPFLOW_SWEEP_CLOCK
__device__ long long g_sweep_clk[4096 * 8];
#endif
template <int MODE, bool SHARE>
__device__ __forceinline__ void sweep_job(const SweepParams &p, const int lin)
{
#ifdef ICPFLOW_SWEEP_CLOCK
    const long long dbgW0 = wall_clock64(), dbgC0 = clock64();
    long long dbgC1 = 0, dbgC2 = 0;
    int dbgRounds = 0, dbgChunks = 0;
#endif
    __shared__ double red[(kSweepBlock / kWave) * kPartial];
    extern __shared__ __attribute__((aligned(16))) float keyLds[];
    int job = (lin / (8 * p.qblocks)) * 8 + (lin & 7);
    int qb = (lin >> 3) % p.qblocks;
    if (MODE == SWEEP_SCORE && p.prune) {
        const int padded = (p.njobs + 7) & ~7;
        qb = lin / padded;
        job = lin % padded;
        if (p.listMode == 2) {
            const int cnt = *p.listCount;
            qb = lin / cnt;
            job = p.list[lin % cnt];
        }
    }
    if (MODE == SWEEP_CHECK && p.initSum != nullptr) {
        const int pairs = p.njobs >> 1;
        const int half = ((pairs + 7) / 8) * 8 * p.qblocks;
        const int l = lin < half ? lin : lin - half;
        const int k = (l / (8 * p.qblocks)) * 8 + (l & 7);
        qb = (l >> 3) % p.qblocks;
        if (k >= pairs) return;
        job = k * 2 + (lin < half ? 1 : 0);
    }
    if (job >= p.njobs) return;
    const int listedAs = job;
    int b = (MODE == SWEEP_SCORE) ? job / p.subCount : job >> 1;
    const int sub = (MODE == SWEEP_SCORE) ? p.subBegin + job % p.subCount : (job & 1);
    if (SHARE && p.pairTab != nullptr && (MODE == SWEEP_SCORE || p.active == nullptr)) {
        const bool bw = (MODE == SWEEP_SCORE) ? (sub & 1) : (MODE == SWEEP_EVAL ? sub == 1 : false);
        const int e = p.pairTab[b * 4 + (MODE == SWEEP_EVAL ? 2 : 0) + (bw ? 1 : 0)];
        const int blocks = (p.shareCount != nullptr) ? ((e >> 8) & 255) : (e & 255);
        if (qb >= blocks) {
            const int bb = e >> 16;
            double *rec = p.partial + ((size_t)((MODE == SWEEP_SCORE) ? bb * 12 + sub : bb * 2 + sub) * p.qblocks + qb) * kPartial;
            if (threadIdx.x < kPartial) rec[threadIdx.x] = 0.0;
            if (MODE == SWEEP_SCORE && p.listMode == 1)
                for (int k = kPartial + threadIdx.x; k < p.qblocks * kPartial; k += kSweepBlock) rec[k] = 0.0;
            return;
        }
    }
    if (p.pairOrder != nullptr) b = p.pairOrder[b];
    job = (MODE == SWEEP_SCORE) ? b * 12 + sub : b * 2 + sub;
    if (MODE == SWEEP_SCORE && p.listMode == 1) {
        double *rec = p.partial + ((size_t)job * p.qblocks + 1) * kPartial;
        for (int k = threadIdx.x; k < (p.qblocks - 1) * kPartial; k += kSweepBlock) rec[k] = 0.0;
    }
    if (MODE == SWEEP_SCORE && p.prune == 1 && p.occBits != nullptr && qb > 0) {
        const double seen = __hip_atomic_load(p.accum + job, __ATOMIC_RELAXED, __HIP_MEMORY_SCOPE_AGENT);
        if (seen == __builtin_huge_val()) {
            double *rec = p.partial + ((size_t)job * p.qblocks + qb) * kPartial;
            if (threadIdx.x < kPartial) rec[threadIdx.x] = threadIdx.x == 0 ? __builtin_huge_val() : 0.0;
            return;
        }
    }
    if (MODE == SWEEP_CHECK && sub == 0 && p.initSum != nullptr) {
        const double t = p.initSum[b];
        if (t - t == 0.0 && (p.active == nullptr || p.active[b] != 0)) return;
    }
    const bool backward = (MODE == SWEEP_SCORE) ? (sub & 1) : (MODE == SWEEP_EVAL ? sub == 1 : false);
    const bool sw = p.swap != nullptr && p.swap[b] != 0;
    const int na = (sw ? p.lenC : p.lenA)[b], nc = (sw ? p.lenA : p.lenC)[b];
    const float *as = p.Asoa + (size_t)b * 3 * p.NP16, *cs = p.Csoa + (size_t)b * 3 * p.NP16;
    int naE = na, ncE = nc;
    if (MODE == SWEEP_EVAL && sw) {
        const float *t = as; as = cs; cs = t;
        naE = nc; ncE = na;
    }
    const float *qs = backward ? cs : as, *ts = backward ? as : cs, *ks = ts;
    if (MODE == SWEEP_EVAL) {
        const float *st = p.srcT + (size_t)b * 3 * p.NP16;
        if (!backward) qs = st;
        else { ts = st; ks = as; }
    }
    const int nq = backward ? ncE : naE, nt = backward ? naE : ncE;
    double *out = p.partial + ((size_t)job * p.qblocks + qb) * kPartial;
    const int lane = threadIdx.x & (kWave - 1), wave = threadIdx.x >> 6;
    __shared__ float boundSh;
    __shared__ int prunedSh;
    const bool off = MODE != SWEEP_SCORE && p.active != nullptr && p.active[b] == 0;
    const int nqb = (nq + kSweepBlock - 1) / kSweepBlock;
    const bool fullScan = SHARE && !off && p.shareCount != nullptr && nq > 0 && nqb <= kSweepFullQb && nt >= kSweepFullScanMinNt && p.qblocks >= 2 * nqb;
    const int shares = fullScan ? min(p.qblocks / nqb, kSweepShares) : 1;
    const int qi = fullScan ? qb % nqb : qb, si = fullScan ? qb / nqb : 0;
    if (fullScan && qb >= nqb && qb < shares * nqb) {
        if (threadIdx.x < kPartial) out[threadIdx.x] = 0.0;
        out = p.partial + ((size_t)job * p.qblocks + qi) * kPartial;
    } else
    if (off || qb * kSweepBlock >= nq) {
        if (threadIdx.x < kPartial) out[threadIdx.x] = 0.0;
        return;
    }
    if (MODE == SWEEP_SCORE && threadIdx.x == 0) prunedSh = 0;
    if (MODE == SWEEP_SCORE && p.prune && !fullScan) {
        __shared__ int leave;
        __shared__ double scanSum[12];
        if (wave == 0 && p.qblocks <= kWave) {
            const int q = min(lane, p.qblocks - 1);
            double v[11];
#pragma unroll
            for (int u = 0; u < 11; ++u) {
                const int sc = u == 0 ? 0 : u + 1;
                v[u] = (u == 0 || p.prune == 2) ? p.partial[((size_t)(b * 12 + sc) * p.qblocks + q) * kPartial] : 0.0;
            }
            if (p.boundBoth) {
                const double v1 = p.partial[((size_t)(b * 12 + 1) * p.qblocks + q) * kPartial];
                double t = 0.0;
                for (int qq = 0; qq < p.qblocks; ++qq) t += __shfl(v1, qq, kWave);
                if (lane == 0) scanSum[1] = t;
            }
#pragma unroll
            for (int u = 0; u < 11; ++u) {
                if (u > 0 && p.prune != 2) break;
                double t = 0.0;
                for (int qq = 0; qq < p.qblocks; ++qq) t += __shfl(v[u], qq, kWave);
                if (lane == 0) scanSum[u == 0 ? 0 : u + 1] = t;
            }
        }
        __syncthreads();
        if (threadIdx.x == 0) {
            double f0 = 0.0;
            if (p.qblocks <= kWave) f0 = scanSum[0];
            else for (int q = 0; q < p.qblocks; ++q) f0 += p.partial[((size_t)(b * 12 + 0) * p.qblocks + q) * kPartial];
            float bound = (float)f0 / (float)na;
            if (p.boundBoth) {
                double b0 = 0.0;
                if (p.qblocks <= kWave) b0 = scanSum[1];
                else for (int q = 0; q < p.qblocks; ++q) b0 += p.partial[((size_t)(b * 12 + 1) * p.qblocks + q) * kPartial];
                bound = fminf(bound, (float)b0 / (float)nc);
            }
            boundSh = bound;
            if (p.prune == 2) {
                bool othersOut = true;
                for (int k = 1; k < 6; ++k) {
                    double fk = 0.0, bk = 0.0;
                    if (p.qblocks <= kWave) { fk = scanSum[2 * k]; bk = scanSum[2 * k + 1]; }
                    else for (int q = 0; q < p.qblocks; ++q) {
                        fk += p.partial[((size_t)(b * 12 + 2 * k) * p.qblocks + q) * kPartial];
                        bk += p.partial[((size_t)(b * 12 + 2 * k + 1) * p.qblocks + q) * kPartial];
                    }
                    const float sk = fminf((float)fk / (float)na, (float)bk / (float)nc);
                    othersOut = othersOut && (sk > bound * 1.0001f);
                }
                leave = othersOut ? 1 : 0;
            } else {
                const double seen = __hip_atomic_load(p.accum + job, __ATOMIC_RELAXED, __HIP_MEMORY_SCOPE_AGENT);
                const float low = (float)(seen / (double)(float)(backward ? nc : na));
                leave = low > bound * 1.0001f ? 1 : 0;
            }
            if (leave) {
                out[0] = __builtin_huge_val();
                for (int k = 1; k < kPartial; ++k) out[k] = 0.0;
            }
        }
        __syncthreads();
        if (leave) return;
        if (p.prune == 1 && p.occBits != nullptr && sub != 1 && qb == 0 && p.listMode != 2) {
            __shared__ int occCount[kSweepBlock / kWave];
            __shared__ int occLeave;
            const float *t3 = p.cand + ((size_t)b * 6 + (sub >> 1)) * 3;
            const float ptx = t3[0], pty = t3[1], ptz = t3[2];
            const int role = backward ? 0 : 1;
            const float *hdr = p.occHdr + ((size_t)b * 2 + role) * 8;
            const uint32_t *bits = p.occBits + ((size_t)b * 2 + role) * kOccRings * kOccWords;
            const float gox = hdr[0], goy = hdr[1], goz = hdr[2], ginv = hdr[3], hlb = hdr[4];
            const int gnx = __float_as_int(hdr[5]), gny = __float_as_int(hdr[6]), gnz = __float_as_int(hdr[7]);
            int cnt = 0;
            if (gnx > 0) {
                for (int i = threadIdx.x; i < nq; i += kSweepBlock) {
                    float x = qs[i], y = qs[p.NP16 + i], z = qs[2 * p.NP16 + i];
                    if (!backward) { x += ptx; y += pty; z += ptz; }
                    else { x -= ptx; y -= pty; z -= ptz; }
                    const float ux = floorf((x - gox) * ginv), uy = floorf((y - goy) * ginv), uz = floorf((z - goz) * ginv);
                    const bool inside = ux >= 0.f && ux < (float)gnx && uy >= 0.f && uy < (float)gny && uz >= 0.f && uz < (float)gnz;
                    const bool finite = fabsf(x) < 1e30f && fabsf(y) < 1e30f && fabsf(z) < 1e30f;
                    int level = (finite && !inside) ? kOccRings : 0;
                    if (inside) {
                        const int c = ((int)ux * gny + (int)uy) * gnz + (int)uz;
#pragma unroll
                        for (int ring = 0; ring < kOccRings; ++ring)
                            level += ((bits[ring * kOccWords + (c >> 5)] >> (c & 31)) & 1u) == 0u ? 1 : 0;
                    }
                    cnt += level;
                }
            }
            cnt = wave_sum(cnt);
            if (lane == 0) occCount[wave] = cnt;
            __syncthreads();
            if (threadIdx.x == 0) {
                int tot = 0;
                for (int w = 0; w < kSweepBlock / kWave; ++w) tot += occCount[w];
                const float low = ((float)tot * hlb * 0.999f) / (float)(backward ? nc : na);
                occLeave = low > boundSh * 1.0001f ? 1 : 0;
#ifdef ICPFLOW_OCC_STATS
                atomicAdd(&g_occStats[0], 1ull); if (occLeave) atomicAdd(&g_occStats[1], 1ull);
                if (!occLeave && b < 1024) atomicAdd(&g_occPair[b], 1u);
                atomicAdd(&g_occStats[2], (unsigned long long)tot); atomicAdd(&g_occStats[3], (unsigned long long)nq);
                const float ratio = low / boundSh;
                atomicAdd(&g_occStats[4 + min(7, max(0, (int)(ratio * 4.0f)))], 1ull);
#endif
                if (occLeave) {
                    out[0] = __builtin_huge_val();
                    for (int k = 1; k < kPartial; ++k) out[k] = 0.0;
                    atomicAdd(p.accum + job, __builtin_huge_val());
                }
            }
            __syncthreads();
            if (occLeave) return;
        }
    }
    if (MODE == SWEEP_SCORE && p.listMode == 1) {
        if (threadIdx.x == 0) p.list[atomicAdd(p.listCount, 1)] = listedAs;
        return;
    }
    __shared__ float poseSh[16];
    if (MODE == SWEEP_CHECK) {
        if (sub == 1 && p.poseB == nullptr) {
            if (wave == 0) {
                const int n = pose_stop_iteration_wave(p.fused, lane);
                if (lane == 0) {
                    float M[16];
                    final_pose(p.fused, b, n, M);
#pragma unroll
                    for (int k = 0; k < 16; ++k) poseSh[k] = M[k];
                }
            }
        } else if (threadIdx.x < 16) {
            poseSh[threadIdx.x] = ((sub == 0 ? p.poseA : p.poseB) + (size_t)b * 16)[threadIdx.x];
        }
        __syncthreads();
    }
    float tx = 0.f, ty = 0.f, tz = 0.f;
    if (MODE == SWEEP_SCORE) {
        const float *t3 = p.cand + ((size_t)b * 6 + (sub >> 1)) * 3;
        tx = t3[0]; ty = t3[1]; tz = t3[2];
    }
    const int axis = p.axis[b];
    float dirX = 0.f, dirY = 0.f;
    if (axis >= 3) sort_dir(axis, dirX, dirY);
    const float tu = sort_key_of(axis, dirX, dirY, tx, ty, tz);
// ... 121 lines not shown
                __syncthreads();
#pragma unroll
                for (int w = 0; w < kSweepBlock / kWave; ++w) best = fminf(best, shareBest[w][lane]);
                __syncthreads();
            }
#ifdef ICPFLOW_SWEEP_CLOCK
            ++dbgRounds; dbgChunks = ce - cb;
#endif
            cb = min(cb, k0); ce = max(ce, k1);
            const float worst = wave_max_uniform(live ? best : 0.f);
            const float proven = r * shrink;
            if (MODE == SWEEP_SCORE && p.prune == 1) {
                const float sb = sqrtf(best), pr = proven * 0.99999f;
                const float lbLane = !live ? 0.f : (sb < pr ? sb : (sb != sb ? sb : pr));
                const float L = wave_sum(lbLane) * 0.99999f;
                if (lane == 0 && L > lbAdded && (!sharedWindow || wave == 0)) atomicAdd(p.accum + job, (double)(L - lbAdded));
                if (L > lbAdded) lbAdded = L;
                const bool done = worst <= proven * proven || (cb == 0 && ce == np16);
                if (!done) {
                    double seen = 0.0;
                    if (lane == 0) seen = __hip_atomic_load(p.accum + job, __ATOMIC_RELAXED, __HIP_MEMORY_SCOPE_AGENT);
                    const float low = __int_as_float(__builtin_amdgcn_readfirstlane(
                        __float_as_int((float)(seen / (double)(float)(backward ? nc : na)))));
                    bool leaveNow = low > boundSh * 1.0001f;
                    if (sharedWindow) {
                        if (threadIdx.x == 0) shareLeave = leaveNow ? 1 : 0;
                        __syncthreads();
                        leaveNow = shareLeave != 0;
                        __syncthreads();
                    }
                    if (leaveNow) {
                        if (lane == 0) prunedSh = 1;
                        break;
                    }
                }
            }
            if (worst <= proven * proven || (cb == 0 && ce == np16)) break;
            const float rPrev = r;
            r = (worst < kInf) ? sqrtf(worst) * (MODE == SWEEP_EVAL ? 1.001f : 1.000002f) : r * 4.0f;
#ifndef ICPFLOW_SWEEP_GROWTH
#define ICPFLOW_SWEEP_GROWTH 2.0f
#endif
            if (MODE == SWEEP_SCORE && p.prune == 1) r = fminf(r, rPrev * ICPFLOW_SWEEP_GROWTH);
        }
    }
#ifdef ICPFLOW_SWEEP_CLOCK
    dbgC2 = clock64();
#ifndef ICPFLOW_SWEEP_CLOCK_MODE
#define ICPFLOW_SWEEP_CLOCK_MODE 1
#endif
    if (MODE == ICPFLOW_SWEEP_CLOCK_MODE && threadIdx.x == 0) {
        const int slot = (MODE == SWEEP_SCORE ? job : b * 2 + sub) & 4095;
        long long *o = g_sweep_clk + slot * 8;
        const long long now = wall_clock64();
        if (now > o[1]) { o[0] = dbgW0; o[1] = now; o[2] = dbgC1 - dbgC0; o[3] = dbgC2 - dbgC1; o[4] = dbgRounds; o[5] = nt; o[6] = nq; o[7] = qb; }
    }
#endif
    double v[kPartial];
#pragma unroll
    for (int k = 0; k < kPartial; ++k) v[k] = 0.0;
    if (live && nt > 0 && (!sharedWindow || wave == 0)) {
        const float d = sqrtf(best);
        v[0] = (double)d;
        if (MODE == SWEEP_EVAL) {
            v[1] = (d < p.thres) ? 1.0 : 0.0;
            if (!backward) { v[2] = qx; v[3] = qy; v[4] = qz; v[5] = ox; v[6] = oy; v[7] = oz; }
        }
    }
    constexpr int NV = (MODE == SWEEP_EVAL) ? kPartial : 1;
#pragma unroll
    for (int k = 0; k < NV; ++k) v[k] = wave_sum(v[k]);
    if (lane == 0)
        for (int k = 0; k < NV; ++k) red[wave * kPartial + k] = v[k];
    __syncthreads();
    if (threadIdx.x < kPartial) {
        double ssum = 0.0;
        if (threadIdx.x < NV)
            for (int w = 0; w < kSweepBlock / kWave; ++w) ssum += red[w * kPartial + threadIdx.x];
        if (MODE == SWEEP_SCORE && prunedSh != 0 && threadIdx.x == 0) ssum = __builtin_huge_val();
        out[threadIdx.x] = ssum;
    }
}

template <int MODE, bool SHARE = false>
__global__ __launch_bounds__(kSweepBlock) void sweep_scan_kernel(SweepParams p)
{
    sweep_job<MODE, SHARE>(p, (int)blockIdx.x);
}

template <int MODE, bool SHARE = false>
__global__ __launch_bounds__(kSweepBlock) void sweep_list_kernel(SweepParams p)
{
    const int entries = *p.listCount * p.qblocks;
    for (int e = (int)blockIdx.x; e < entries; e += (int)gridDim.x) {
        sweep_job<MODE, SHARE>(p, e);
        __syncthreads();
    }
}

__global__ void transform_soa_kernel(const float *__restrict__ soa, const int32_t *__restrict__ len,
                                     const float *__restrict__ pose, int NP16, float *__restrict__ out,
                                     const float *__restrict__ soaSwapped, const uint8_t *__restrict__ swap)
{
    const int b = blockIdx.y, k = blockIdx.x * blockDim.x + threadIdx.x;
    if (k >= NP16) return;
    const float *in = ((swap != nullptr && swap[b] != 0) ? soaSwapped : soa) + (size_t)b * 3 * NP16;
    float *o = out + (size_t)b * 3 * NP16;
    float x = kInf, y = kInf, z = kInf;
    if (k < len[b]) {
        const Affine a = affine_from_pose(pose + (size_t)b * 16);
        affine_apply(a, in[k], in[NP16 + k], in[2 * NP16 + k], x, y, z);
    }
    o[k] = x; o[NP16 + k] = y; o[2 * NP16 + k] = z;
}

#ifdef ICPFLOW_SWEEP_CLOCK
extern "C" int icpflow_debug_sweep_clk(long long *out32768)
{
    return (int)hipMemcpyFromSymbol(out32768, HIP_SYMBOL(g_sweep_clk), sizeof(long long) * 32768);
}
#endif
int sweep_qblocks(int maxRows) { return (maxRows + kSweepBlock - 1) / kSweepBlock; }

__global__ void sweep_pair_table_kernel(const int32_t *__restrict__ lenA, const int32_t *__restrict__ lenC,
                                        const uint8_t *__restrict__ swap, const int32_t *__restrict__ pairOrder, int B,
                                        int qblocks, int32_t *__restrict__ tab)
{
    const int k = blockIdx.x * blockDim.x + threadIdx.x;
    if (k >= B) return;
    const int b = pairOrder != nullptr ? pairOrder[k] : k;
    const bool sw = swap != nullptr && swap[b] != 0;
    const int na = (sw ? lenC : lenA)[b], nc = (sw ? lenA : lenC)[b];
    const int nqs[4] = {na, nc, lenA[b], lenC[b]}, nts[4] = {nc, na, lenC[b], lenA[b]};
#pragma unroll
    for (int d = 0; d < 4; ++d) {
        const int nq = nqs[d], nt = nts[d];
        const int nqb = (nq + kSweepBlock - 1) / kSweepBlock;
        const bool fullScan = nq > 0 && nqb <= kSweepFullQb && nt >= kSweepFullScanMinNt && qblocks >= 2 * nqb;
        const int shares = fullScan ? min(qblocks / nqb, kSweepShares) : 1;
        tab[k * 4 + d] = (b << 16) | (min(shares * nqb, 255) << 8) | min(nqb, 255);
    }
}

hipError_t launch_sweep_pair_table(const int32_t *lenA, const int32_t *lenC, const uint8_t *swap, const int32_t *pairOrder,
                                   int B, int N, int32_t *tab, hipStream_t s)
{
    if (B > 32767 || sweep_qblocks(N) > 255) return hipErrorInvalidValue;
    hipLaunchKernelGGL(sweep_pair_table_kernel, dim3((B + 255) / 256), dim3(256), 0, s, lenA, lenC, swap, pairOrder, B,
                       sweep_qblocks(N), tab);
    return hipGetLastError();
}

template <int MODE>
static hipError_t launch_sweep(SweepParams p, hipStream_t s)
{
    p.NP16 = (p.N + kChunk - 1) / kChunk * kChunk;
    p.qblocks = sweep_qblocks(p.N);
    p.r0 = 0.15f;
#ifndef ICPFLOW_NO_SWEEP_SHARE
    p.shareWindows = 1;
#endif
#ifdef ICPFLOW_NO_SWEEP_SHARE
    p.shareCount = nullptr;
#endif
    if (p.N < kSweepFullScanMinTargets || p.shareBest == nullptr) p.shareCount = nullptr;
    if (p.shareCount != nullptr && !p.shareClean) {
        const hipError_t me = hipMemsetAsync(p.shareCount, 0, (size_t)(MODE == SWEEP_SCORE ? (p.njobs / p.subCount) * 12 : p.njobs) * kSweepFullQb * sizeof(int), s);
        if (me != hipSuccess) return me;
    }
    const int groups = (MODE == SWEEP_CHECK && p.initSum != nullptr) ? 2 * ((p.njobs / 2 + 7) / 8) : (p.njobs + 7) / 8;
    const size_t lds = (size_t)((p.NP16 < kSweepStage ? p.NP16 : kSweepStage) * 33 / 32 + 1) * sizeof(float);
    const int total = groups * 8 * p.qblocks;
    if (MODE == SWEEP_SCORE && p.listMode == 1) {
        const int first = groups * 8;
        if (p.shareWindows != 0 && p.N >= kSweepFullScanMinTargets && p.njobs <= 12 * 700)
            hipLaunchKernelGGL((sweep_scan_kernel<MODE, true>), dim3((unsigned)first), dim3(kSweepBlock), lds, s, p);
        else
            hipLaunchKernelGGL((sweep_scan_kernel<MODE, false>), dim3((unsigned)first), dim3(kSweepBlock), lds, s, p);
        return hipGetLastError();
    }
    if (MODE == SWEEP_SCORE && p.listMode == 2) {
        const int wgs = total < 8 * 256 ? total : 8 * 256;
        if (p.shareWindows != 0 && p.N >= kSweepFullScanMinTargets && p.njobs <= 12 * 700)
            hipLaunchKernelGGL((sweep_list_kernel<MODE, true>), dim3((unsigned)wgs), dim3(kSweepBlock), lds, s, p);
        else
            hipLaunchKernelGGL((sweep_list_kernel<MODE, false>), dim3((unsigned)wgs), dim3(kSweepBlock), lds, s, p);
        return hipGetLastError();
    }
    if (p.shareWindows != 0 && p.N >= kSweepFullScanMinTargets && p.njobs <= 12 * 700)
        hipLaunchKernelGGL((sweep_scan_kernel<MODE, true>), dim3((unsigned)total), dim3(kSweepBlock), lds, s, p);
    else
        hipLaunchKernelGGL((sweep_scan_kernel<MODE, false>), dim3((unsigned)total), dim3(kSweepBlock), lds, s, p);
    return hipGetLastError();
}

constexpr int kOccBlock = 256;
__device__ __forceinline__ uint32_t occ_shifted(const uint32_t *in, int w, int sh, bool up)
{
    const int q = sh >> 5, r = sh & 31;
    if (up) {
        const int a = w - q;
        const uint32_t lo = a >= 0 ? in[a] : 0u, lo1 = a - 1 >= 0 ? in[a - 1] : 0u;
        return r == 0 ? lo : ((lo << r) | (lo1 >> (32 - r)));
    }
    const int a = w + q;
    const uint32_t hi = a < kOccWords ? in[a] : 0u, hi1 = a + 1 < kOccWords ? in[a + 1] : 0u;
    return r == 0 ? hi : ((hi >> r) | (hi1 << (32 - r)));
}

__global__ __launch_bounds__(kOccBlock) void occ_build_kernel(const float *__restrict__ Xsoa, const float *__restrict__ Ysoa,
                                                            int NP16, float *__restrict__ hdrOut, uint32_t *__restrict__ bitsOut)
{
    __shared__ uint32_t bitsA[kOccWords], bitsB[kOccWords];
    __shared__ float red[6 * (kOccBlock / kWave)];
    __shared__ float hd[8];
    const int b = blockIdx.x, which = blockIdx.y, tid = threadIdx.x, lane = tid & (kWave - 1), wave = tid >> 6;
    const float *px = (which == 0 ? Xsoa : Ysoa) + (size_t)b * 3 * NP16, *py = px + NP16, *pz = py + NP16;
    for (int k = tid; k < kOccWords; k += kOccBlock) bitsA[k] = 0u;
    float mn[3] = {kInf, kInf, kInf}, mx[3] = {-kInf, -kInf, -kInf};
    for (int i = tid; i < NP16; i += kOccBlock) {
        const float x = px[i], y = py[i], z = pz[i];
        if (fabsf(x) < 1e30f && fabsf(y) < 1e30f && fabsf(z) < 1e30f) {
            mn[0] = fminf(mn[0], x); mn[1] = fminf(mn[1], y); mn[2] = fminf(mn[2], z);
            mx[0] = fmaxf(mx[0], x); mx[1] = fmaxf(mx[1], y); mx[2] = fmaxf(mx[2], z);
        }
    }
#pragma unroll
    for (int a = 0; a < 3; ++a) {
#pragma unroll
        for (int o = kWave / 2; o > 0; o >>= 1) {
            mn[a] = fminf(mn[a], __shfl_xor(mn[a], o, kWave));
            mx[a] = fmaxf(mx[a], __shfl_xor(mx[a], o, kWave));
        }
        if (lane == 0) { red[wave * 6 + a] = mn[a]; red[wave * 6 + 3 + a] = mx[a]; }
    }
    __syncthreads();
    if (tid == 0) {
        float lo[3], hi[3];
        for (int a = 0; a < 3; ++a) {
            lo[a] = kInf; hi[a] = -kInf;
            for (int w = 0; w < kOccBlock / kWave; ++w) { lo[a] = fminf(lo[a], red[w * 6 + a]); hi[a] = fmaxf(hi[a], red[w * 6 + 3 + a]); }
        }
        int n[3] = {0, 0, 0};
        float h = 0.125f;
        if (lo[0] <= hi[0]) {
            for (int grow = 0; grow < 64; ++grow) {
                bool fits = true;
                long long cells = 1;
                for (int a = 0; a < 3; ++a) {
                    const float e = (hi[a] - lo[a]) / h;
                    if (!(e < 30000.f)) { fits = false; break; }
                    n[a] = (int)e + 2 + 2 * kOccRings;
                    cells *= n[a];
                }
                if (fits && cells <= (long long)kOccWords * 32) break;
                h *= 1.25f; n[0] = 0;
            }
        }
        if (n[0] <= 0) n[0] = n[1] = n[2] = 0;
        hd[0] = lo[0] - kOccRings * h; hd[1] = lo[1] - kOccRings * h; hd[2] = lo[2] - kOccRings * h;
        float big = 0.f;
        for (int a = 0; a < 3; ++a) big = fmaxf(big, fmaxf(fabsf(lo[a]), fabsf(hi[a])));
        if (!(big * 2.4e-7f / h < 0.005f)) n[0] = n[1] = n[2] = 0;
        hd[3] = 1.0f / h; hd[4] = 0.98f * h;
        hd[5] = __int_as_float(n[0]); hd[6] = __int_as_float(n[1]); hd[7] = __int_as_float(n[2]);
    }
    __syncthreads();
    const float gox = hd[0], goy = hd[1], goz = hd[2], ginv = hd[3];
    const int gnx = __float_as_int(hd[5]), gny = __float_as_int(hd[6]), gnz = __float_as_int(hd[7]);
    if (gnx > 0) {
        for (int i = tid; i < NP16; i += kOccBlock) {
            const float x = px[i], y = py[i], z = pz[i];
            if (!(fabsf(x) < 1e30f && fabsf(y) < 1e30f && fabsf(z) < 1e30f)) continue;
            const int cx = min(max((int)floorf((x - gox) * ginv), kOccRings), gnx - 1 - kOccRings);
            const int cy = min(max((int)floorf((y - goy) * ginv), kOccRings), gny - 1 - kOccRings);
            const int cz = min(max((int)floorf((z - goz) * ginv), kOccRings), gnz - 1 - kOccRings);
            const int c = (cx * gny + cy) * gnz + cz;
            atomicOr(&bitsA[c >> 5], 1u << (c & 31));
        }
    }
    __syncthreads();
    const int strides[3] = {1, gnz, gny * gnz};
    uint32_t *in = bitsA, *outb = bitsB;
    uint32_t *bo = bitsOut + ((size_t)b * 2 + which) * kOccRings * kOccWords;
    for (int ring = 0; ring < kOccRings; ++ring) {
        for (int a = 0; a < 3; ++a) {
            if (gnx > 0)
                for (int w = tid; w < kOccWords; w += kOccBlock) outb[w] = in[w] | occ_shifted(in, w, strides[a], true) | occ_shifted(in, w, strides[a], false);
            __syncthreads();
            uint32_t *t = in; in = outb; outb = t;
        }
        for (int k = tid; k < kOccWords; k += kOccBlock) bo[ring * kOccWords + k] = gnx > 0 ? in[k] : 0u;
    }
    if (tid < 8) hdrOut[((size_t)b * 2 + which) * 8 + tid] = hd[tid];
}

hipError_t launch_occupancy(const GridScratch *grid, int B, int N, hipStream_t s)
{
    if (grid->occHdr == nullptr || grid->occBits == nullptr || grid->sortXsoa == nullptr || grid->sortYsoa == nullptr) return hipSuccess;
    const int NP16 = (N + kChunk - 1) / kChunk * kChunk;
    hipLaunchKernelGGL(occ_build_kernel, dim3(B, 2), dim3(kOccBlock), 0, s, grid->sortXsoa, grid->sortYsoa, NP16, grid->occHdr, grid->occBits);
    return hipGetLastError();
}

hipError_t launch_sweep_score(const GridScratch *grid, const int32_t *lenA, const int32_t *lenC, const uint8_t *swap,
                              int B, int N, const float *cand, double *partial, hipStream_t s)
{
    SweepParams p{};
    p.Asoa = grid->sortXsoa; p.Csoa = grid->sortYsoa; p.lenA = lenA; p.lenC = lenC; p.swap = swap;
    p.axis = grid->axis; p.cand = cand; p.N = N; p.njobs = B * 12; p.partial = partial;
    p.subBegin = 0; p.subCount = 12;
    p.shareBest = grid->shareBest; p.shareCount = grid->shareCount; p.shareClean = grid->shareCountClean; p.pairOrder = grid->pairOrder; p.pairTab = grid->pairTab;
    return launch_sweep<SWEEP_SCORE>(p, s);
}

hipError_t launch_sweep_score_pruned(const GridScratch *grid, const int32_t *lenA, const int32_t *lenC,
                                     const uint8_t *swap, int B, int N, const float *cand, double *partial,
                                     double *accum, hipStream_t s)
{
    SweepParams p{};
    p.Asoa = grid->sortXsoa; p.Csoa = grid->sortYsoa; p.lenA = lenA; p.lenC = lenC; p.swap = swap;
    p.axis = grid->axis; p.cand = cand; p.N = N; p.partial = partial; p.accum = accum;
    if (grid->occReady) { p.occHdr = grid->occHdr; p.occBits = grid->occBits; }
    p.shareBest = grid->shareBest; p.shareCount = grid->shareCount; p.shareClean = grid->shareCountClean; p.pairOrder = grid->pairOrder; p.pairTab = grid->pairTab;
    if (grid->occReady) {
        p.njobs = B * 2; p.subBegin = 0; p.subCount = 2; p.prune = 0;
        hipError_t e2 = launch_sweep<SWEEP_SCORE>(p, s);
        if (e2 != hipSuccess) return e2;
        p.njobs = B * 10; p.subBegin = 2; p.subCount = 10; p.prune = 1; p.boundBoth = 1;
#ifndef ICPFLOW_SCORE_LIST_MIN_JOBS
#define ICPFLOW_SCORE_LIST_MIN_JOBS 65536
#endif
        if (grid->sweepTicket != nullptr && grid->scoreList != nullptr &&
            (long long)B * 10 * sweep_qblocks(N) >= ICPFLOW_SCORE_LIST_MIN_JOBS) {
            p.list = grid->scoreList; p.listCount = grid->sweepTicket;
            p.listMode = 1;
            const hipError_t e3 = launch_sweep<SWEEP_SCORE>(p, s);
            if (e3 != hipSuccess) return e3;
            p.listMode = 2;
        }
        return launch_sweep<SWEEP_SCORE>(p, s);
    }
    p.njobs = B; p.subBegin = 0; p.subCount = 1; p.prune = 0;
    hipError_t e = launch_sweep<SWEEP_SCORE>(p, s);
    if (e != hipSuccess) return e;
    p.njobs = B * 11; p.subBegin = 1; p.subCount = 11; p.prune = 1;
    return launch_sweep<SWEEP_SCORE>(p, s);
}

hipError_t launch_sweep_eval(const GridScratch *grid, const int32_t *len1, const int32_t *len2, int B, int N,
                             const float *pose, float thres, float *srcT, double *partial, hipStream_t s,
                             const uint8_t *swap, const uint8_t *active)
{
    SweepParams p{};
    p.active = active;
    p.Asoa = grid->sortXsoa; p.Csoa = grid->sortYsoa; p.lenA = len1; p.lenC = len2; p.axis = grid->axis;
    p.swap = swap;
    p.poseA = pose; p.thres = thres; p.srcT = srcT; p.N = N; p.njobs = B * 2; p.partial = partial;
    p.shareBest = grid->shareBest; p.shareCount = grid->shareCount; p.shareClean = grid->shareCountClean; p.pairOrder = grid->pairOrder; p.pairTab = grid->pairTab;
    const int NP16 = (N + kChunk - 1) / kChunk * kChunk;
    hipLaunchKernelGGL(transform_soa_kernel, dim3((NP16 + 255) / 256, B), dim3(256), 0, s, grid->sortXsoa, len1, pose,
                       NP16, srcT, grid->sortYsoa, swap);
    return launch_sweep<SWEEP_EVAL>(p, s);
}

hipError_t launch_sweep_check(const GridScratch *grid, const float *X, const float *Y, const int32_t *lenA,
                              const int32_t *lenC, const uint8_t *swap, int B, int N, const float *poseInit,
                              const float *poseFinal, double *partial, hipStream_t s, const PoseSource *fused,
                              const uint8_t *active, const double *initSum)
{
    SweepParams p{};
    p.active = active;
    p.initSum = initSum;
    if (poseFinal == nullptr) {
        if (fused == nullptr) return hipErrorInvalidValue;
        p.fused = *fused;
    }
    p.Asoa = grid->sortYsoa;
    p.Csoa = grid->sortYsoa; p.lenA = lenA; p.lenC = lenC; p.swap = swap; p.axis = grid->axis;
    p.sortX = (const float4 *)grid->sortX; p.X = X; p.Y = Y; p.poseA = poseInit; p.poseB = poseFinal;
    p.rawSorted = grid->presorted; p.N = N; p.njobs = B * 2; p.partial = partial;
    p.shareBest = grid->shareBest; p.shareCount = grid->shareCount; p.shareClean = grid->shareCountClean; p.pairOrder = grid->pairOrder; p.pairTab = grid->pairTab;
    return launch_sweep<SWEEP_CHECK>(p, s);
}

hipError_t launch_scan_score(const float *A, const float *C, const int32_t *lenA, const int32_t *lenC,
                             const uint8_t *swap, int B, int N, const float *cand, double *partial,
                             hipStream_t s)
{
    ScanParams p{};
    p.A = A; p.C = C; p.lenA = lenA; p.lenC = lenC; p.swap = swap; p.N = N;
    p.njobs = B * 12; p.cand = cand; p.partial = partial;
    p.subBegin = 0; p.subCount = 12;
    return launch_scan<MODE_SCORE>(p, N, B, s);
}

constexpr int kScoreSplit = 2;
int score_qblocks(int maxRows) { return (maxRows + kScanBlock / kScoreSplit - 1) / (kScanBlock / kScoreSplit); }

hipError_t launch_scan_score_pruned(const float *A, const float *C, const int32_t *lenA, const int32_t *lenC,
                                    const uint8_t *swap, int B, int N, const float *cand, double *partial,
                                    double *accum, hipStream_t s, bool accumCleared)
{
    if (!accumCleared) {
        hipError_t e = hipMemsetAsync(accum, 0, (size_t)B * 12 * sizeof(double), s);
        if (e != hipSuccess) return e;
    }
    ScanParams p{};
    p.A = A; p.C = C; p.lenA = lenA; p.lenC = lenC; p.swap = swap; p.N = N;
    p.cand = cand; p.partial = partial; p.accum = accum;
    p.qblocks = score_qblocks(N);
    p.split = kScoreSplit;
    p.njobs = B; p.subBegin = 0; p.subCount = 1; p.prune = 0;
    hipLaunchKernelGGL((nn_scan_kernel<1, MODE_SCORE>), dim3((unsigned)(((p.njobs + 7) / 8) * 8 * p.qblocks)),
                       dim3(kScanBlock), 0, s, p);
    p.njobs = B * 11; p.subBegin = 1; p.subCount = 11; p.prune = 1;
    hipLaunchKernelGGL((nn_scan_kernel<1, MODE_SCORE>), dim3((unsigned)(((p.njobs + 7) & ~7) * p.qblocks)),
                       dim3(kScanBlock), 0, s, p);
    return hipGetLastError();
}

hipError_t launch_scan_check(const float *A, const float *C, const int32_t *lenA, const int32_t *lenC,
                             const uint8_t *swap, int B, int N, const float *poseInit,
                             const float *poseFinal, double *partial, hipStream_t s)
{
    ScanParams p{};
    p.A = A; p.C = C; p.lenA = lenA; p.lenC = lenC; p.swap = swap; p.N = N;
    p.njobs = B * 2; p.poseA = poseInit; p.poseB = poseFinal; p.partial = partial;
    return launch_scan<MODE_CHECK>(p, N, B, s);
}

hipError_t launch_scan_eval(const float *A, const float *C, const int32_t *lenA, const int32_t *lenC,
                            int B, int N, const float *pose, float thres, double *partial, hipStream_t s)
{
    ScanParams p{};
    p.A = A; p.C = C; p.lenA = lenA; p.lenC = lenC; p.swap = nullptr; p.N = N;
    p.njobs = B * 2; p.poseA = pose; p.thres = thres; p.partial = partial;
    return launch_scan<MODE_EVAL>(p, N, B, s);
}

hipError_t launch_scan_nn(const float *Qp, const float *Tp, int B, int NQ, int NT, int strideQ,
                          int strideT, const int32_t *lenQ, const int32_t *lenT, int sqrt_dist,
                          int64_t *idx, float *dist, hipStream_t s)
{
    ScanParams p{};
    p.A = Qp; p.C = Tp; p.lenA = lenQ; p.lenC = lenT; p.N = NQ; p.NT = NT;
    p.strideQ = strideQ; p.strideT = strideT; p.njobs = B; p.idx = idx; p.dist = dist;
    p.sqrt_dist = sqrt_dist;
    return launch_scan<MODE_NN>(p, NQ, 1 << 30, s);
}

}

#ifdef ICPFLOW_OCC_STATS
extern "C" int icpflow_debug_occ_pairs(unsigned int *out1024, int reset)
{
    (void)hipDeviceSynchronize();
    const int rc = (int)hipMemcpyFromSymbol(out1024, HIP_SYMBOL(icpflow::g_occPair), sizeof(icpflow::g_occPair));
    if (reset) {
        static unsigned int z[1024];
        (void)hipMemcpyToSymbol(HIP_SYMBOL(icpflow::g_occPair), z, sizeof(z));
    }
    return rc;
}
// ... 12 lines not shown
```

icp_flow_amd/csrc/pose.hip:

```cpp
#include "common.hpp"
#include "kernels.hpp"
#include "posefuse.hpp"

namespace icpflow {

__device__ __forceinline__ double partial_total(const double *partial, int job, int qblocks, int k)
{
    double s = 0.0;
    const double *base = partial + (size_t)job * qblocks * kPartial + k;
    if (qblocks <= 4) {
        double v[4];
#pragma unroll
        for (int u = 0; u < 4; ++u) v[u] = base[(size_t)min(u, qblocks - 1) * kPartial];
#pragma unroll
        for (int u = 0; u < 4; ++u)
            if (u < qblocks) s += v[u];
        return s;
    }
    for (int q0 = 0; q0 < qblocks; q0 += 8) {
        double v[8];
#pragma unroll
        for (int u = 0; u < 8; ++u) v[u] = base[(size_t)min(q0 + u, qblocks - 1) * kPartial];
#pragma unroll
        for (int u = 0; u < 8; ++u)
            if (q0 + u < qblocks) s += v[u];
    }
    return s;
}

__global__ __launch_bounds__(kWave) void score_pick_kernel(const double *__restrict__ partial, int qblocks,
                                                           const int32_t *__restrict__ lenA,
                                                           const int32_t *__restrict__ lenC,
                                                           const uint8_t *__restrict__ swap,
                                                           const float *__restrict__ cand, int B,
                                                           float *__restrict__ Tinit, double *__restrict__ initSum)
{
    const int b = blockIdx.x, lane = threadIdx.x;
    const bool sw = swap != nullptr && swap[b] != 0;
    const float na = (float)(sw ? lenC[b] : lenA[b]);
    const float nc = (float)(sw ? lenA[b] : lenC[b]);
    float mean = 0.f;
    double total = 0.0;
    if (lane < 2 * kCand) {
        total = partial_total(partial, b * 12 + lane, qblocks, 0);
        mean = (float)total / ((lane & 1) ? nc : na);
    }
    int pick = 0;
    float best = 0.f;
    for (int k = 0; k < kCand; ++k) {
        const float sc = fminf(__shfl(mean, 2 * k, kWave), __shfl(mean, 2 * k + 1, kWave));
        if (k == 0 || sc < best) { best = sc; pick = k; }
    }
    if (initSum != nullptr && lane == 2 * pick) initSum[b] = total;
    if (lane < 16) {
        const float *t = cand + ((size_t)b * kCand + pick) * 3;
        float v = (lane % 5 == 0) ? 1.f : 0.f;
        if (lane == 3) v = t[0];
        if (lane == 7) v = t[1];
        if (lane == 11) v = t[2];
        Tinit[(size_t)b * 16 + lane] = v;
    }
}

hipError_t launch_score_pick(const double *partial, int qblocks, const int32_t *lenA,
                             const int32_t *lenC, const uint8_t *swap, const float *cand, int B,
                             float *Tinit, hipStream_t s, double *initSum)
{
    hipLaunchKernelGGL(score_pick_kernel, dim3(B), dim3(kWave), 0, s, partial, qblocks, lenA, lenC, swap, cand, B,
                       Tinit, initSum);
    return hipGetLastError();
}

__global__ void compose_kernel(const IcpState *__restrict__ st, const float *__restrict__ init, int B,
                               float *__restrict__ M, const IcpCtrl *__restrict__ ctrl, int32_t *__restrict__ iters)
{
    const int b = blockIdx.x * blockDim.x + threadIdx.x;
    if (b == 0 && iters != nullptr) *iters = ctrl->error ? -1 : ctrl->iters;
    if (b >= B) return;
    float A[16];
    for (int i = 0; i < 3; ++i) {
        for (int j = 0; j < 3; ++j) A[i * 4 + j] = st[b].R[j * 3 + i];
        A[i * 4 + 3] = st[b].T[i];
    }
    A[12] = A[13] = A[14] = 0.f; A[15] = 1.f;
    if (ctrl != nullptr && ctrl->error) A[0] = __int_as_float(0x7fc00000);
    const float *I = init + (size_t)b * 16;
    float *o = M + (size_t)b * 16;
    for (int i = 0; i < 4; ++i)
        for (int j = 0; j < 4; ++j) {
            float acc = A[i * 4 + 0] * I[0 * 4 + j];
            acc = fmaf(A[i * 4 + 1], I[1 * 4 + j], acc);
            acc = fmaf(A[i * 4 + 2], I[2 * 4 + j], acc);
            acc = fmaf(A[i * 4 + 3], I[3 * 4 + j], acc);
            o[i * 4 + j] = acc;
        }
}

hipError_t launch_compose(const IcpState *state, const float *init, int B, float *M, hipStream_t s,
                          const IcpCtrl *ctrl, int32_t *iters)
{
    hipLaunchKernelGGL(compose_kernel, dim3((B + 127) / 128), dim3(128), 0, s, state, init, B, M, ctrl, iters);
    return hipGetLastError();
}

#ifdef ICPFLOW_REUSE_STATS
__device__ unsigned long long g_reuseStats[4];
#endif
__global__ void select_kernel(const double *__restrict__ partial, int qblocks,
                              const int32_t *__restrict__ lenA, const int32_t *__restrict__ lenC,
                              const uint8_t *__restrict__ swap, const float *__restrict__ init,
                              const float *__restrict__ M, int B, int invertSwapped, float *__restrict__ out,
                              PoseSource fused, int32_t *__restrict__ iters, const double *__restrict__ initSum,
                              const uint8_t *__restrict__ active)
{
    const int b = blockIdx.x * blockDim.x + threadIdx.x;
    int n = 0;
    if (M == nullptr) {
        n = pose_stop_iteration_wave(fused, threadIdx.x & (kWave - 1));
        if (b == 0 && iters != nullptr) *iters = fused.ctrl->error ? -1 : n;
    }
    if (b >= B) return;
    float Mf[16];
    if (M == nullptr) final_pose(fused, b, n, Mf);
    const bool sw = swap != nullptr && swap[b] != 0;
    const float na = (float)(sw ? lenC[b] : lenA[b]);
    double s0 = 0.0;
    bool reuse = false;
    if (initSum != nullptr && (active == nullptr || active[b] != 0)) {
        s0 = initSum[b];
        reuse = s0 - s0 == 0.0;
    }
    if (!reuse) s0 = partial_total(partial, b * 2 + 0, qblocks, 0);
#ifdef ICPFLOW_REUSE_STATS
    atomicAdd(&g_reuseStats[reuse ? 0 : (initSum != nullptr ? 1 : 2)], 1ull);
#endif
    const float e0 = (float)s0 / na;
    const float e1 = (float)partial_total(partial, b * 2 + 1, qblocks, 0) / na;
    const float *src = (e1 >= e0) ? init + (size_t)b * 16 : (M != nullptr ? M + (size_t)b * 16 : Mf);
#ifdef ICPFLOW_REUSE_STATS
    if (e1 >= e0) atomicAdd(&g_reuseStats[3], 1ull);
#endif
    float P[16];
    for (int k = 0; k < 16; ++k) P[k] = src[k];
    if (sw && invertSwapped) {
        const double a = P[0], bb = P[1], c = P[2], d = P[4], e = P[5], f = P[6], g = P[8], h = P[9],
                     i = P[10];
        const double tx = P[3], ty = P[7], tz = P[11];
        const double c00 = e * i - f * h, c01 = c * h - bb * i, c02 = bb * f - c * e;
        const double c10 = f * g - d * i, c11 = a * i - c * g, c12 = c * d - a * f;
        const double c20 = d * h - e * g, c21 = bb * g - a * h, c22 = a * e - bb * d;
        const double det = a * c00 + bb * c10 + c * c20;
        const double r = 1.0 / det;
        const double I00 = c00 * r, I01 = c01 * r, I02 = c02 * r;
        const double I10 = c10 * r, I11 = c11 * r, I12 = c12 * r;
        const double I20 = c20 * r, I21 = c21 * r, I22 = c22 * r;
        P[0] = (float)I00; P[1] = (float)I01; P[2] = (float)I02;
        P[4] = (float)I10; P[5] = (float)I11; P[6] = (float)I12;
        P[8] = (float)I20; P[9] = (float)I21; P[10] = (float)I22;
        P[3] = (float)(-(I00 * tx + I01 * ty + I02 * tz));
        P[7] = (float)(-(I10 * tx + I11 * ty + I12 * tz));
        P[11] = (float)(-(I20 * tx + I21 * ty + I22 * tz));
        P[12] = P[13] = P[14] = 0.f; P[15] = 1.f;
    }
    float *o = out + (size_t)b * 16;
    for (int k = 0; k < 16; ++k) o[k] = P[k];
}

hipError_t launch_select(const double *partial, int qblocks, const int32_t *lenA, const int32_t *lenC,
                         const uint8_t *swap, const float *init, const float *M, int B, int invertSwapped,
                         float *out, hipStream_t s, const PoseSource *fused, int32_t *iters, const double *initSum,
                         const uint8_t *active)
{
    if (M == nullptr && fused == nullptr) return hipErrorInvalidValue;
    hipLaunchKernelGGL(select_kernel, dim3((B + 127) / 128), dim3(128), 0, s, partial, qblocks, lenA, lenC,
                       swap, init, M, B, invertSwapped, out, fused ? *fused : PoseSource{}, iters, initSum, active);
    return hipGetLastError();
}

__global__ __launch_bounds__(kWave) void eval_epilogue_kernel(const double *__restrict__ partial, int qblocks,
                                                              const int32_t *__restrict__ len1,
                                                              const int32_t *__restrict__ len2,
                                                              const float *__restrict__ T, int B,
                                                              float *__restrict__ errors, float *__restrict__ inliers,
                                                              float *__restrict__ ratios, float *__restrict__ ious,
                                                              float *__restrict__ translations,
                                                              float *__restrict__ rotations)
{
    const int b = blockIdx.x, lane = threadIdx.x;
    double tot = 0.0;
    if (lane < 2 * kPartial) tot = partial_total(partial, b * 2 + lane / kPartial, qblocks, lane % kPartial);
    const float n1 = (float)len1[b], n2 = (float)len2[b];
    const float n12 = (float)(len1[b] + len2[b]);
    const float sum1 = (float)__shfl(tot, 0, kWave), sum2 = (float)__shfl(tot, kPartial, kWave);
    const float in1 = (float)__shfl(tot, 1, kWave), in2 = (float)__shfl(tot, kPartial + 1, kWave);
    float moved[3], orig[3];
#pragma unroll
    for (int k = 0; k < 3; ++k) {
        moved[k] = (float)__shfl(tot, 2 + k, kWave) / n1;
        orig[k] = (float)__shfl(tot, 5 + k, kWave) / n1;
    }
    if (lane != 0) return;
    errors[b * 2 + 0] = sum1 / n1;
    errors[b * 2 + 1] = sum2 / n2;
    inliers[b * 2 + 0] = in1;
    inliers[b * 2 + 1] = in2;
    ratios[b * 2 + 0] = in1 / n1;
    ratios[b * 2 + 1] = in2 / n2;
    ious[b * 2 + 0] = in1 / (n12 - in2);
    ious[b * 2 + 1] = in2 / (n12 - in1);
    for (int k = 0; k < 3; ++k) translations[b * 3 + k] = moved[k] - orig[k];
    const float *M = T + (size_t)b * 16;
    const float pi = 3.14159265358979323846f;
    rotations[b * 3 + 0] = (atan2f(M[4], M[0]) * 180.0f) / pi;
    rotations[b * 3 + 1] = (asinf(-M[8]) * 180.0f) / pi;
    rotations[b * 3 + 2] = (atan2f(M[9], M[10]) * 180.0f) / pi;
}

hipError_t launch_eval_epilogue(const double *partial, int qblocks, const int32_t *len1,
                                const int32_t *len2, const float *T, int B, float *errors,
                                float *inliers, float *ratios, float *ious, float *translations,
                                float *rotations, hipStream_t s)
{
    hipLaunchKernelGGL(eval_epilogue_kernel, dim3(B), dim3(kWave), 0, s, partial, qblocks, len1, len2, T, B, errors,
                       inliers, ratios, ious, translations, rotations);
    return hipGetLastError();
}

__global__ void transform_points_kernel(const float4 *xyz, const float *__restrict__ pose, int N, float4 *out)
{
    const int b = blockIdx.y;
    const int i = blockIdx.x * blockDim.x + threadIdx.x;
    if (i >= N) return;
    const Affine a = affine_from_pose(pose + (size_t)b * 16);
    const float4 p = xyz[(size_t)b * N + i];
    float4 o;
    affine_apply(a, p.x, p.y, p.z, o.x, o.y, o.z);
    o.w = p.w;
    out[(size_t)b * N + i] = o;
}

hipError_t launch_transform_points(const float *xyz, const float *pose, int B, int N, float *out,
                                   hipStream_t s)
{
    hipLaunchKernelGGL(transform_points_kernel, dim3((N + 255) / 256, B), dim3(256), 0, s,
                       (const float4 *)xyz, pose, N, (float4 *)out);
    return hipGetLastError();
}

// ... 176 lines not shown
```

include/icpflow_hip.h:

```cpp
#ifndef ICPFLOW_HIP_H
#define ICPFLOW_HIP_H

#include <stddef.h>
#include <stdint.h>

#ifdef __cplusplus
extern "C" {
#endif

#define ICPFLOW_VERSION 214

#define ICPFLOW_OK 0
#define ICPFLOW_E_ARG (-1)
#define ICPFLOW_E_WORKSPACE (-2)
#define ICPFLOW_E_LIMIT (-3)
#define ICPFLOW_E_HOSTMEM (-4)

#define ICPFLOW_STOP_REFERENCE 0
#define ICPFLOW_STOP_PER_PAIR 1

typedef void *icpflow_stream_t;

int icpflow_version(void);
const char *icpflow_last_error(void);
const char *icpflow_build_info(void);

#define ICPFLOW_SEARCH_AUTO 0
#define ICPFLOW_SEARCH_SCAN 1
#define ICPFLOW_SEARCH_GRID 2
#define ICPFLOW_SEARCH_SWEEP 3
#define ICPFLOW_ARITH_FP64 0
#define ICPFLOW_ARITH_FP32_REFERENCE 1
#define ICPFLOW_OPT_NO_SORTED_VOTE (1u << 0)
#define ICPFLOW_OPT_NO_SIDE_STREAM (1u << 1)
#define ICPFLOW_OPT_NO_EVAL_SWEEP (1u << 2)
#define ICPFLOW_OPT_NO_CHECK_SWEEP (1u << 3)
#define ICPFLOW_OPT_NO_SCORE_SWEEP (1u << 4)
#define ICPFLOW_OPT_NO_SCORE_PRUNE (1u << 5)
#define ICPFLOW_OPT_NO_TEAMS (1u << 6)
#define ICPFLOW_OPT_NO_SPECULATIVE (1u << 7)
#define ICPFLOW_OPT_NO_ADAPTIVE_WINDOWS (1u << 8)
#define ICPFLOW_OPT_NO_PERSISTENT (1u << 9)
#define ICPFLOW_OPT_NO_HELPERS (1u << 10)
#define ICPFLOW_OPT_TEAMS_HALF_GPU (1u << 11)
#define ICPFLOW_OPT_NO_SHARED_SCANS (1u << 12)
#define ICPFLOW_OPT_NO_STAGE_OVERLAP (1u << 13)
#define ICPFLOW_OPT_NO_VOTE_LIST (1u << 14)
#define ICPFLOW_OPT_NO_CHECK_REUSE (1u << 15)
#define ICPFLOW_OPT_NO_SCORE_PREBOUND (1u << 16)
#define ICPFLOW_OPT_TWO_LAUNCH (1u << 17)
#define ICPFLOW_OPT_NO_DIR_KEYS (1u << 18)

typedef struct icpflow_profile icpflow_profile_t;

typedef struct icpflow_options {
    size_t struct_size;
    int icp_search;
    int icp_arith;
    unsigned flags;
    icpflow_profile_t *profile;
    uint32_t *d_vote_bins_u32;
    const float *d_icp_init_R;
    const float *d_icp_init_T;
    float *d_icp_history;
    int icp_allow_reflection;
    int icp_estimate_scale;
    float *d_icp_scale;
    const float *d_icp_init_s;
    const uint8_t *d_pair_active;
} icpflow_options_t;

size_t icpflow_workspace_bytes(int B, int N, int Lx, int Ly, int Lz);

int icpflow_hist_vote(const float *d_X, const float *d_Y, int B, int NX, int NY,
                      float min_x, float min_y, float min_z,
                      float max_x, float max_y, float max_z,
                      int len_x, int len_y, int len_z,
                      float *d_bins, icpflow_stream_t stream);

int icpflow_hist_peaks(const float *d_bins, int B, int len_x, int len_y, int len_z,
                       int k, int kernel_size, float *d_votes, int64_t *d_idx,
                       void *d_ws, size_t ws_bytes, icpflow_stream_t stream);

int icpflow_nn_batch(const float *d_Q, const float *d_T, int B, int NQ, int NT,
                     int q_stride, int t_stride, const int32_t *d_len_q,
                     const int32_t *d_len_t, int sqrt_dist, int64_t *d_idx,
                     float *d_dist, icpflow_stream_t stream);

int icpflow_transform_points(const float *d_xyz, const float *d_pose, int B, int N,
                             float *d_out, icpflow_stream_t stream);

int icpflow_count_valid(const float *d_pts, int B, int N, int32_t *d_len,
                        icpflow_stream_t stream);

int icpflow_estimate_init_pose(const float *d_src, const float *d_dst, int B, int N,
                               const float *d_edges_x, int len_x,
                               const float *d_edges_y, int len_y,
                               const float *d_edges_z, int len_z,
                               float decode_shift, float *d_T_out,
                               void *d_ws, size_t ws_bytes, icpflow_stream_t stream,
                               const icpflow_options_t *opt);

int icpflow_icp(const float *d_X, const float *d_Y, const float *d_pre_pose, int B, int N,
                double thres, int max_iterations, double relative_rmse_thr, int stop_mode,
                float *d_R, float *d_T, float *d_rmse, int32_t *d_iters,
                int32_t *d_converged, void *d_ws, size_t ws_bytes,
                icpflow_stream_t stream, const icpflow_options_t *opt);

int icpflow_apply_icp(const float *d_src, const float *d_dst, const float *d_init,
                      int B, int N, double thres_dist, int max_iterations,
                      double relative_rmse_thr, int stop_mode, float *d_T_out,
                      int32_t *d_iters, void *d_ws, size_t ws_bytes,
                      icpflow_stream_t stream, const icpflow_options_t *opt);

int icpflow_hist_icp(const float *d_src, const float *d_dst, int B, int N,
                     const float *d_edges_x, int len_x,
                     const float *d_edges_y, int len_y,
                     const float *d_edges_z, int len_z,
                     float decode_shift, double thres_dist, int max_iterations,
                     double relative_rmse_thr, int stop_mode, float *d_T_out,
                     int32_t *d_iters, void *d_ws, size_t ws_bytes,
                     icpflow_stream_t stream, const icpflow_options_t *opt);

int icpflow_hist_icp_many(int K, const float *const *d_src, const float *const *d_dst, const int *B, int N,
                          const float *d_edges_x, int len_x, const float *d_edges_y, int len_y,
                          const float *d_edges_z, int len_z, float decode_shift, double thres_dist,
                          int max_iterations, double relative_rmse_thr, int stop_mode, float *const *d_T_out,
                          int32_t *const *d_iters, void *const *d_ws, const size_t *ws_bytes,
                          icpflow_stream_t stream, const icpflow_options_t *opt);

int icpflow_match_eval(const float *d_pcd1, const float *d_pcd2, const float *d_T,
                       int B, int N, double thres_dist, float *d_errors,
                       float *d_inliers, float *d_ratios, float *d_ious,
                       float *d_translations, float *d_rotations, void *d_ws,
// ... 181 lines not shown
```

Baseline: 403,900.

## Fold score-pick and final select into sweep kernels via per-pair last-block tickets

Adds a per-pair atomic ticket so the last block finishing a pair's sweep-score or sweep-check work runs the candidate pick or final pose select inline. This removes the separate score_pick and select kernel launches along with their dependent launch gaps. The pick sum is stored in a new buffer that is threaded through the phased API. The shared pick and select logic moves into a common header. The cost is extra atomics and fences per block, plus serial tail work done by a single block per pair.

```diff
diff --git a/icp_flow_amd/_lib.py b/icp_flow_amd/_lib.py
--- a/icp_flow_amd/_lib.py
+++ b/icp_flow_amd/_lib.py
@@ -108,6 +108,7 @@
              "no_stage_overlap": 1 << 13, "no_vote_list": 1 << 14, "no_check_reuse": 1 << 15, "no_score_prebound": 1 << 16,
              "two_launch": 1 << 17,
              "no_dir_keys": 1 << 18}
+OPT_FLAGS_TAILS = {"no_score_one_launch": 1 << 19, "no_select_fold": 1 << 20}
 
 
 class Options(ctypes.Structure):
@@ -203,7 +204,7 @@
 
 def _env_default_flags():
     f = 0
-    for name, bit in OPT_FLAGS.items():
+    for name, bit in {**OPT_FLAGS, **OPT_FLAGS_TAILS}.items():
         if os.environ.get("ICPFLOW_" + name.upper(), "0") not in ("0", ""):
             f |= bit
     return f
@@ -242,7 +243,8 @@
     if pair_active is not None:
         cur["pair_active"] = pair_active
     for k, v in switches.items():
-        cur["flags"] = (cur["flags"] | OPT_FLAGS[k]) if v else (cur["flags"] & ~OPT_FLAGS[k])
+        bit = OPT_FLAGS_TAILS[k] if k in OPT_FLAGS_TAILS else OPT_FLAGS[k]
+        cur["flags"] = (cur["flags"] | bit) if v else (cur["flags"] & ~bit)
     stack = getattr(_tls, "stack", None)
     if stack is None:
         stack = _tls.stack = []
diff --git a/icp_flow_amd/csrc/api.hip b/icp_flow_amd/csrc/api.hip
--- a/icp_flow_amd/csrc/api.hip
+++ b/icp_flow_amd/csrc/api.hip
@@ -166,6 +166,9 @@
     int32_t *icpSplit = nullptr;
     bool initSumValid = false;
     int *ticketScratch = nullptr;
+    int *pairTicket = nullptr;
+    double *pickSum = nullptr;
+    const double *initSumAt = nullptr;
     size_t accumBytes = 0;
     size_t bytes = 0;
     static bool shareScratch(int B, int N) { return N >= 2048 && (size_t)B * 12 * kSweepShareSlots * 256 * 4 <= ((size_t)64 << 20); }
@@ -194,8 +197,10 @@
             partial = (double *)take(b * 12 * qb * kPartial * 8);
             scoreAccum = (double *)take(b * 12 * 8);
             ticketScratch = (int *)take(256);
+            pairTicket = (int *)take(b * 4);
             if (shareScratch(B, N)) grid.shareCount = (int *)take(b * 12 * kSweepShareSlots * 4);
-            accumBytes = up(b * 12 * 8) + up(256) + (shareScratch(B, N) ? up(b * 12 * kSweepShareSlots * 4) : 0);
+            accumBytes = up(b * 12 * 8) + up(256) + up(b * 4) + (shareScratch(B, N) ? up(b * 12 * kSweepShareSlots * 4) : 0);
+            pickSum = (double *)take(b * 8);
         }
         Tinit = (float *)take(b * 16 * 4);
         M = (float *)take(b * 16 * 4);
@@ -269,7 +274,7 @@
         return fail(ICPFLOW_E_ARG, "%s: options.icp_search must be 0..3 (got %d)", fn, opt->icp_search);
     if (opt->icp_arith != ICPFLOW_ARITH_FP64 && opt->icp_arith != ICPFLOW_ARITH_FP32_REFERENCE)
         return fail(ICPFLOW_E_ARG, "%s: options.icp_arith must be 0 or 1 (got %d)", fn, opt->icp_arith);
-    if (opt->flags >> 19) return fail(ICPFLOW_E_ARG, "%s: unknown option flags 0x%x", fn, opt->flags);
+    if (opt->flags >> 21) return fail(ICPFLOW_E_ARG, "%s: unknown option flags 0x%x", fn, opt->flags);
     o.search = opt->icp_search;
     o.arith = opt->icp_arith;
     o.flags = opt->flags;
@@ -421,9 +426,12 @@
     }
     if (sweepCheck) {
         PoseSource ps{w.state, w.ctrl, historyPending ? w.history : nullptr, init, B, maxIter};
-        const double *initSum = (initSumValid && search->presorted && o.on(ICPFLOW_OPT_NO_CHECK_REUSE)) ? w.scoreAccum : nullptr;
+        const double *initSum = (initSumValid && search->presorted && o.on(ICPFLOW_OPT_NO_CHECK_REUSE))
+                                    ? (w.initSumAt != nullptr ? w.initSumAt : w.scoreAccum) : nullptr;
+        const bool fold = search->pairTicket != nullptr && o.on(ICPFLOW_OPT_NO_SELECT_FOLD);
         ICPFLOW_TRY(launch_sweep_check(search, src, dst, w.lenA, w.lenC, swap, B, N, init, nullptr, w.partial, s, &ps, o.pairActive,
-                                       initSum));
+                                       initSum, fold ? Tout : nullptr, iters, invertSwapped));
+        if (fold) return 0;
         ICPFLOW_TRY(launch_select(w.partial, sweep_qblocks(N), w.lenA, w.lenC, swap, init, nullptr, B, invertSwapped,
                                   Tout, s, &ps, iters, initSum, o.pairActive));
         return 0;
@@ -474,12 +482,16 @@
                 w.grid.occReady = 1;
             }
         }
-        if (o.on(ICPFLOW_OPT_NO_SCORE_PRUNE))
-            ICPFLOW_TRY(launch_sweep_score_pruned(&w.grid, w.lenA, w.lenC, swap, B, N, w.cand, w.partial, w.scoreAccum, s));
-        else
+        bool picked = false;
+        if (o.on(ICPFLOW_OPT_NO_SCORE_PRUNE)) {
+            const bool one = o.on(ICPFLOW_OPT_NO_SCORE_ONE_LAUNCH);
+            ICPFLOW_TRY(launch_sweep_score_pruned(&w.grid, w.lenA, w.lenC, swap, B, N, w.cand, w.partial, w.scoreAccum, s,
+                                                  one ? Tout : nullptr, w.pickSum, &picked));
+        } else
             ICPFLOW_TRY(launch_sweep_score(&w.grid, w.lenA, w.lenC, swap, B, N, w.cand, w.partial, s));
-        ICPFLOW_TRY(launch_score_pick(w.partial, sweep_qblocks(N), w.lenA, w.lenC, swap, w.cand, B, Tout, s, w.scoreAccum));
+        if (!picked) ICPFLOW_TRY(launch_score_pick(w.partial, sweep_qblocks(N), w.lenA, w.lenC, swap, w.cand, B, Tout, s, w.scoreAccum));
         w.initSumValid = true;
+        w.initSumAt = picked ? w.pickSum : w.scoreAccum;
     } else if (o.on(ICPFLOW_OPT_NO_SCORE_PRUNE)) {
         ICPFLOW_TRY(launch_scan_score_pruned(src, dst, w.lenA, w.lenC, swap, B, N, w.cand, w.partial, w.scoreAccum, s, true));
         ICPFLOW_TRY(launch_score_pick(w.partial, score_qblocks(N), w.lenA, w.lenC, swap, w.cand, B, Tout, s));
@@ -932,7 +944,9 @@
     Workspace w(d_ws, B, N, L);
     if (int r = check_ws(d_ws, ws_bytes, w.bytes)) return r;
     hipStream_t s = (hipStream_t)stream;
-    launch_count_pair(d_src, d_dst, B, N, w.lenA, w.lenC, nullptr, s, w.scoreAccum, (size_t)B * 12 * sizeof(double));
+    launch_count_pair(d_src, d_dst, B, N, w.lenA, w.lenC, nullptr, s, w.scoreAccum, w.accumBytes);
+    w.grid.shareCountClean = 1;
+    w.grid.pairTicket = w.pairTicket;
     return run_init_pose(d_src, d_dst, w, nullptr, B, N, d_edges_x, len_x, d_edges_y, len_y, d_edges_z,
                          len_z, decode_shift, d_T_out, o, s);
 }
@@ -1022,6 +1036,8 @@
     if (phase == 2) {
         w.grid.presorted = carry[0];
         w.grid.shareCountClean = 1;
+        w.grid.pairTicket = w.pairTicket;
+        w.initSumAt = carry[3] == 2 ? w.pickSum : w.scoreAccum;
         int32_t pending = carry[2];
         return run_icp_and_select(d_src, d_dst, w, w.swap, w.Tinit, B, N, thres_dist, max_iterations,
                                   relative_rmse_thr, stop_mode, 1, d_T_out, d_iters, o, s, carry[1] != 0, 2, &pending, carry[3] != 0);
@@ -1070,6 +1086,7 @@
     }
     w.grid.shareCountClean = 1;
     w.grid.sweepTicket = w.ticketScratch;
+    w.grid.pairTicket = w.pairTicket;
     const bool sweepScore = score_by_sweep(N, join != nullptr, o);
     if (int r = run_init_pose(d_src, d_dst, w, w.swap, B, N, d_edges_x, len_x, d_edges_y, len_y, d_edges_z,
                               len_z, decode_shift, w.Tinit, o, s, sweepScore ? join : nullptr,
@@ -1080,7 +1097,7 @@
     if (phase == 1) {
         carry[0] = w.grid.presorted;
         carry[1] = teamPlanned ? 1 : 0;
-        carry[3] = w.initSumValid ? 1 : 0;
+        carry[3] = w.initSumValid ? (w.initSumAt == w.pickSum ? 2 : 1) : 0;
         return run_icp_and_select(d_src, d_dst, w, w.swap, w.Tinit, B, N, thres_dist, max_iterations, relative_rmse_thr,
                                   stop_mode, 1, d_T_out, d_iters, o, s, teamPlanned, 1, &carry[2]);
     }
diff --git a/icp_flow_amd/csrc/kernels.hpp b/icp_flow_amd/csrc/kernels.hpp
--- a/icp_flow_amd/csrc/kernels.hpp
+++ b/icp_flow_amd/csrc/kernels.hpp
@@ -147,13 +147,15 @@
 hipError_t launch_sweep_check(const GridScratch *grid, const float *X, const float *Y, const int32_t *lenA,
                               const int32_t *lenC, const uint8_t *swap, int B, int N, const float *poseInit,
                               const float *poseFinal, double *partial, hipStream_t s, const PoseSource *fused = nullptr,
-                              const uint8_t *active = nullptr, const double *initSum = nullptr);
+                              const uint8_t *active = nullptr, const double *initSum = nullptr,
+                              float *selOut = nullptr, int32_t *selIters = nullptr, int selInvertSwapped = 0);
 hipError_t launch_occupancy(const GridScratch *grid, int B, int N, hipStream_t s);
 hipError_t launch_sweep_score(const GridScratch *grid, const int32_t *lenA, const int32_t *lenC, const uint8_t *swap,
                               int B, int N, const float *cand, double *partial, hipStream_t s);
 hipError_t launch_sweep_score_pruned(const GridScratch *grid, const int32_t *lenA, const int32_t *lenC,
                                      const uint8_t *swap, int B, int N, const float *cand, double *partial,
-                                     double *accum, hipStream_t s);
+                                     double *accum, hipStream_t s, float *pickT = nullptr, double *pickSum = nullptr,
+                                     bool *picked = nullptr);
 hipError_t launch_scan_score(const float *A, const float *C, const int32_t *lenA, const int32_t *lenC,
                              const uint8_t *swap, int B, int N, const float *cand, double *partial,
                              hipStream_t s);
@@ -201,6 +203,7 @@
     int occReady;
     int *sweepTicket;
     int *scoreList;
+    int *pairTicket;
     int presorted;
 };
 int grid_buckets(int N);
diff --git a/icp_flow_amd/csrc/nn.hip b/icp_flow_amd/csrc/nn.hip
--- a/icp_flow_amd/csrc/nn.hip
+++ b/icp_flow_amd/csrc/nn.hip
@@ -2,6 +2,7 @@
 #include "sortdir.hpp"
 #include "kernels.hpp"
 #include "posefuse.hpp"
+#include "pairfold.hpp"
 
 namespace icpflow {
 
@@ -287,6 +288,12 @@
     int listMode;
     int *list, *listCount;
     int boundBoth;
+    int *pairTicket;
+    float *pickT;
+    double *pickSum;
+    float *selOut;
+    int32_t *selIters;
+    int selInvertSwapped;
 };
 
 #ifdef ICPFLOW_OCC_STATS
@@ -319,7 +326,7 @@
 __device__ long long g_sweep_clk[4096 * 8];
 #endif
 template <int MODE, bool SHARE>
-__device__ __forceinline__ void sweep_job(const SweepParams &p, const int lin)
+__device__ __forceinline__ void sweep_job(const SweepParams &p, const int lin, int &whoK, int &whoB)
 {
 #ifdef ICPFLOW_SWEEP_CLOCK
     const long long dbgW0 = wall_clock64(), dbgC0 = clock64();
@@ -350,6 +357,7 @@
         job = k * 2 + (lin < half ? 1 : 0);
     }
     if (job >= p.njobs) return;
+    whoK = (MODE == SWEEP_SCORE) ? job / p.subCount : job >> 1;
     const int listedAs = job;
     int b = (MODE == SWEEP_SCORE) ? job / p.subCount : job >> 1;
     const int sub = (MODE == SWEEP_SCORE) ? p.subBegin + job % p.subCount : (job & 1);
@@ -359,6 +367,7 @@
         const int blocks = (p.shareCount != nullptr) ? ((e >> 8) & 255) : (e & 255);
         if (qb >= blocks) {
             const int bb = e >> 16;
+            whoB = bb;
             double *rec = p.partial + ((size_t)((MODE == SWEEP_SCORE) ? bb * 12 + sub : bb * 2 + sub) * p.qblocks + qb) * kPartial;
             if (threadIdx.x < kPartial) rec[threadIdx.x] = 0.0;
             if (MODE == SWEEP_SCORE && p.listMode == 1)
@@ -367,6 +376,7 @@
         }
     }
     if (p.pairOrder != nullptr) b = p.pairOrder[b];
+    whoB = b;
     job = (MODE == SWEEP_SCORE) ? b * 12 + sub : b * 2 + sub;
     if (MODE == SWEEP_SCORE && p.listMode == 1) {
         double *rec = p.partial + ((size_t)job * p.qblocks + 1) * kPartial;
@@ -481,7 +491,7 @@
         }
         __syncthreads();
         if (leave) return;
-        if (p.prune == 1 && p.occBits != nullptr && sub != 1 && qb == 0 && p.listMode != 2) {
+        if (p.prune == 1 && p.occBits != nullptr && sub != 1 && qb == 0 && p.listMode < 2) {
             __shared__ int occCount[kSweepBlock / kWave];
             __shared__ int occLeave;
             const float *t3 = p.cand + ((size_t)b * 6 + (sub >> 1)) * 3;
@@ -769,10 +779,138 @@
     }
 }
 
-template <int MODE, bool SHARE = false>
+template <int MODE, bool SHARE>
+__device__ __forceinline__ void sweep_pair_tail(const SweepParams &p, const int k, const int b)
+{
+    __shared__ int tailLast;
+    __threadfence();
+    __syncthreads();
+    if (threadIdx.x == 0) {
+        const int before = __hip_atomic_fetch_add(p.pairTicket + b, 1, __ATOMIC_ACQ_REL, __HIP_MEMORY_SCOPE_AGENT);
+        tailLast = before == 2 * p.qblocks - 1 ? 1 : 0;
+        if (tailLast) __hip_atomic_store(p.pairTicket + b, 0, __ATOMIC_RELAXED, __HIP_MEMORY_SCOPE_AGENT);
+    }
+    __syncthreads();
+    if (!tailLast) return;
+    __threadfence();
+    const int lane = threadIdx.x & (kWave - 1), wave = threadIdx.x >> 6;
+    if (MODE == SWEEP_CHECK) {
+        if (wave == 0) {
+            const int n = pose_stop_iteration_wave(p.fused, lane);
+            if (lane == 0) {
+                if (b == 0 && p.selIters != nullptr) *p.selIters = p.fused.ctrl->error ? -1 : n;
+                select_pair(p.partial, p.qblocks, p.lenA, p.lenC, p.swap, p.poseA, nullptr, p.selInvertSwapped, p.selOut, p.fused,
+                            p.initSum, p.active, b, n);
+            }
+        }
+        return;
+    }
+    __shared__ float tailBound;
+    __shared__ int tailCount[kSweepBlock / kWave][10];
+    __shared__ int tailGoesOn[10];
+    const bool sw = p.swap != nullptr && p.swap[b] != 0;
+    const int na = (sw ? p.lenC : p.lenA)[b], nc = (sw ? p.lenA : p.lenC)[b];
+    if (threadIdx.x == 0) {
+        double f0 = 0.0, b0 = 0.0;
+        for (int q = 0; q < p.qblocks; ++q)
+            f0 += __hip_atomic_load(p.partial + ((size_t)(b * 12 + 0) * p.qblocks + q) * kPartial, __ATOMIC_RELAXED, __HIP_MEMORY_SCOPE_AGENT);
+        for (int q = 0; q < p.qblocks; ++q)
+            b0 += __hip_atomic_load(p.partial + ((size_t)(b * 12 + 1) * p.qblocks + q) * kPartial, __ATOMIC_RELAXED, __HIP_MEMORY_SCOPE_AGENT);
+        float bound = (float)f0 / (float)na;
+        bound = fminf(bound, (float)b0 / (float)nc);
+        tailBound = bound;
+    }
+    const float *as = p.Asoa + (size_t)b * 3 * p.NP16, *cs = p.Csoa + (size_t)b * 3 * p.NP16;
+    int cnt[10];
+#pragma unroll
+    for (int u = 0; u < 10; ++u) cnt[u] = 0;
+    float tc[5][3];
+#pragma unroll
+    for (int c = 0; c < 5; ++c)
+#pragma unroll
+        for (int a = 0; a < 3; ++a) tc[c][a] = p.cand[((size_t)b * 6 + c + 1) * 3 + a];
+    bool bounded[2] = {false, false};
+    float hlbOf[2] = {0.f, 0.f};
+#pragma unroll
+    for (int dir = 0; dir < 2; ++dir) {
+        const bool backward = dir == 1;
+        const float *qs = backward ? cs : as;
+        const int nq = backward ? nc : na, nt = backward ? na : nc;
+        const int nqb = (nq + kSweepBlock - 1) / kSweepBlock;
+        const bool fullScan = SHARE && p.shareCount != nullptr && nq > 0 && nqb <= kSweepFullQb && nt >= kSweepFullScanMinNt && p.qblocks >= 2 * nqb;
+        if (p.occBits == nullptr || fullScan || nq <= 0) continue;
+        const int role = backward ? 0 : 1;
+        const float *hdr = p.occHdr + ((size_t)b * 2 + role) * 8;
+        const uint32_t *bits = p.occBits + ((size_t)b * 2 + role) * kOccRings * kOccWords;
+        const float gox = hdr[0], goy = hdr[1], goz = hdr[2], ginv = hdr[3];
+        const int gnx = __float_as_int(hdr[5]), gny = __float_as_int(hdr[6]), gnz = __float_as_int(hdr[7]);
+        bounded[dir] = true;
+        hlbOf[dir] = hdr[4];
+        if (gnx <= 0) continue;
+        for (int i = threadIdx.x; i < nq; i += kSweepBlock) {
+            const float x0 = qs[i], y0 = qs[p.NP16 + i], z0 = qs[2 * p.NP16 + i];
+#pragma unroll
+            for (int c = 0; c < 5; ++c) {
+                float x = x0, y = y0, z = z0;
+                if (!backward) { x += tc[c][0]; y += tc[c][1]; z += tc[c][2]; }
+                else { x -= tc[c][0]; y -= tc[c][1]; z -= tc[c][2]; }
+                const float ux = floorf((x - gox) * ginv), uy = floorf((y - goy) * ginv), uz = floorf((z - goz) * ginv);
+                const bool inside = ux >= 0.f && ux < (float)gnx && uy >= 0.f && uy < (float)gny && uz >= 0.f && uz < (float)gnz;
+                const bool finite = fabsf(x) < 1e30f && fabsf(y) < 1e30f && fabsf(z) < 1e30f;
+                int level = (finite && !inside) ? kOccRings : 0;
+                if (inside) {
+                    const int cell = ((int)ux * gny + (int)uy) * gnz + (int)uz;
+#pragma unroll
+                    for (int ring = 0; ring < kOccRings; ++ring)
+                        level += ((bits[ring * kOccWords + (cell >> 5)] >> (cell & 31)) & 1u) == 0u ? 1 : 0;
+                }
+                cnt[c * 2 + dir] += level;
+            }
+        }
+    }
+#pragma unroll
+    for (int u = 0; u < 10; ++u) {
+        const int t = wave_sum(cnt[u]);
+        if (lane == 0) tailCount[wave][u] = t;
+    }
+    __syncthreads();
+    if (threadIdx.x < 10) {
+        const int u = threadIdx.x, dir = u & 1;
+        int tot = 0;
+        for (int w = 0; w < kSweepBlock / kWave; ++w) tot += tailCount[w][u];
+        const float hlb = dir ? hlbOf[1] : hlbOf[0];
+        const float low = ((float)tot * hlb * 0.999f) / (float)(dir ? nc : na);
+        const bool leave = (dir ? bounded[1] : bounded[0]) && low > tailBound * 1.0001f;
+        tailGoesOn[u] = leave ? 0 : 1;
+    }
+    __syncthreads();
+    for (int e = threadIdx.x; e < 10 * p.qblocks * kPartial; e += kSweepBlock) {
+        const int u = e / (p.qblocks * kPartial), r = e % (p.qblocks * kPartial);
+        if (!tailGoesOn[u]) p.partial[((size_t)(b * 12 + 2 + u) * p.qblocks) * kPartial + r] = (r % kPartial) == 0 ? __builtin_huge_val() : 0.0;
+    }
+    SweepParams q = p;
+    q.njobs = (p.njobs / 2) * 10; q.subBegin = 2; q.subCount = 10; q.prune = 1; q.boundBoth = 1; q.listMode = 3;
+    const int padded = (q.njobs + 7) & ~7;
+    for (int u = 0; u < 10; ++u) {
+        if (!tailGoesOn[u]) continue;
+        for (int qb = 0; qb < p.qblocks; ++qb) {
+            int k2 = -1, b2 = -1;
+            __syncthreads();
+            sweep_job<SWEEP_SCORE, SHARE>(q, qb * padded + k * 10 + u, k2, b2);
+        }
+    }
+    __threadfence();
+    __syncthreads();
+    __threadfence();
+    if (wave == 0) score_pick_pair(p.partial, p.qblocks, p.lenA, p.lenC, p.swap, p.cand, b, lane, p.pickT, p.pickSum);
+}
+
+template <int MODE, bool SHARE = false, bool FOLD = false>
 __global__ __launch_bounds__(kSweepBlock) void sweep_scan_kernel(SweepParams p)
 {
-    sweep_job<MODE, SHARE>(p, (int)blockIdx.x);
+    int k = -1, b = -1;
+    sweep_job<MODE, SHARE>(p, (int)blockIdx.x, k, b);
+    if (FOLD && MODE != SWEEP_EVAL && b >= 0) sweep_pair_tail<MODE, SHARE>(p, k, b);
 }
 
 template <int MODE, bool SHARE = false>
@@ -780,7 +918,8 @@
 {
     const int entries = *p.listCount * p.qblocks;
     for (int e = (int)blockIdx.x; e < entries; e += (int)gridDim.x) {
-        sweep_job<MODE, SHARE>(p, e);
+        int k = -1, b = -1;
+        sweep_job<MODE, SHARE>(p, e, k, b);
         __syncthreads();
     }
 }
@@ -874,7 +1013,13 @@
             hipLaunchKernelGGL((sweep_list_kernel<MODE, false>), dim3((unsigned)wgs), dim3(kSweepBlock), lds, s, p);
         return hipGetLastError();
     }
-    if (p.shareWindows != 0 && p.N >= kSweepFullScanMinTargets && p.njobs <= 12 * 700)
+    const bool share = p.shareWindows != 0 && p.N >= kSweepFullScanMinTargets && p.njobs <= 12 * 700;
+    if (MODE != SWEEP_EVAL && p.pairTicket != nullptr) {
+        if (share) hipLaunchKernelGGL((sweep_scan_kernel<MODE == SWEEP_EVAL ? SWEEP_CHECK : MODE, true, true>), dim3((unsigned)total), dim3(kSweepBlock), lds, s, p);
+        else hipLaunchKernelGGL((sweep_scan_kernel<MODE == SWEEP_EVAL ? SWEEP_CHECK : MODE, false, true>), dim3((unsigned)total), dim3(kSweepBlock), lds, s, p);
+        return hipGetLastError();
+    }
+    if (share)
         hipLaunchKernelGGL((sweep_scan_kernel<MODE, true>), dim3((unsigned)total), dim3(kSweepBlock), lds, s, p);
     else
         hipLaunchKernelGGL((sweep_scan_kernel<MODE, false>), dim3((unsigned)total), dim3(kSweepBlock), lds, s, p);
@@ -1001,10 +1146,14 @@
     return launch_sweep<SWEEP_SCORE>(p, s);
 }
 
+#ifndef ICPFLOW_SCORE_LIST_MIN_JOBS
+#define ICPFLOW_SCORE_LIST_MIN_JOBS 65536
+#endif
 hipError_t launch_sweep_score_pruned(const GridScratch *grid, const int32_t *lenA, const int32_t *lenC,
                                      const uint8_t *swap, int B, int N, const float *cand, double *partial,
-                                     double *accum, hipStream_t s)
-{
+                                     double *accum, hipStream_t s, float *pickT, double *pickSum, bool *picked)
+{
+    if (picked != nullptr) *picked = false;
     SweepParams p{};
     p.Asoa = grid->sortXsoa; p.Csoa = grid->sortYsoa; p.lenA = lenA; p.lenC = lenC; p.swap = swap;
     p.axis = grid->axis; p.cand = cand; p.N = N; p.partial = partial; p.accum = accum;
@@ -1012,14 +1161,17 @@
     p.shareBest = grid->shareBest; p.shareCount = grid->shareCount; p.shareClean = grid->shareCountClean; p.pairOrder = grid->pairOrder; p.pairTab = grid->pairTab;
     if (grid->occReady) {
         p.njobs = B * 2; p.subBegin = 0; p.subCount = 2; p.prune = 0;
+        const bool listed = grid->sweepTicket != nullptr && grid->scoreList != nullptr &&
+                            (long long)B * 10 * sweep_qblocks(N) >= ICPFLOW_SCORE_LIST_MIN_JOBS;
+        if (pickT != nullptr && grid->pairTicket != nullptr && !listed) {
+            p.pairTicket = grid->pairTicket; p.pickT = pickT; p.pickSum = pickSum;
+            if (picked != nullptr) *picked = true;
+            return launch_sweep<SWEEP_SCORE>(p, s);
+        }
         hipError_t e2 = launch_sweep<SWEEP_SCORE>(p, s);
         if (e2 != hipSuccess) return e2;
         p.njobs = B * 10; p.subBegin = 2; p.subCount = 10; p.prune = 1; p.boundBoth = 1;
-#ifndef ICPFLOW_SCORE_LIST_MIN_JOBS
-#define ICPFLOW_SCORE_LIST_MIN_JOBS 65536
-#endif
-        if (grid->sweepTicket != nullptr && grid->scoreList != nullptr &&
-            (long long)B * 10 * sweep_qblocks(N) >= ICPFLOW_SCORE_LIST_MIN_JOBS) {
+        if (listed) {
             p.list = grid->scoreList; p.listCount = grid->sweepTicket;
             p.listMode = 1;
             const hipError_t e3 = launch_sweep<SWEEP_SCORE>(p, s);
@@ -1054,7 +1206,7 @@
 hipError_t launch_sweep_check(const GridScratch *grid, const float *X, const float *Y, const int32_t *lenA,
                               const int32_t *lenC, const uint8_t *swap, int B, int N, const float *poseInit,
                               const float *poseFinal, double *partial, hipStream_t s, const PoseSource *fused,
-                              const uint8_t *active, const double *initSum)
+                              const uint8_t *active, const double *initSum, float *selOut, int32_t *selIters, int selInvertSwapped)
 {
     SweepParams p{};
     p.active = active;
@@ -1067,6 +1219,9 @@
     p.Csoa = grid->sortYsoa; p.lenA = lenA; p.lenC = lenC; p.swap = swap; p.axis = grid->axis;
     p.sortX = (const float4 *)grid->sortX; p.X = X; p.Y = Y; p.poseA = poseInit; p.poseB = poseFinal;
     p.rawSorted = grid->presorted; p.N = N; p.njobs = B * 2; p.partial = partial;
+    if (selOut != nullptr && grid->pairTicket != nullptr && poseFinal == nullptr) {
+        p.pairTicket = grid->pairTicket; p.selOut = selOut; p.selIters = selIters; p.selInvertSwapped = selInvertSwapped;
+    }
     p.shareBest = grid->shareBest; p.shareCount = grid->shareCount; p.shareClean = grid->shareCountClean; p.pairOrder = grid->pairOrder; p.pairTab = grid->pairTab;
     return launch_sweep<SWEEP_CHECK>(p, s);
 }
diff --git a/icp_flow_amd/csrc/pairfold.hpp b/icp_flow_amd/csrc/pairfold.hpp
--- /dev/null
+++ b/icp_flow_amd/csrc/pairfold.hpp
@@ -0,0 +1,113 @@
+#pragma once
+#include "common.hpp"
+#include "kernels.hpp"
+#include "posefuse.hpp"
+
+namespace icpflow {
+
+__device__ __forceinline__ double partial_total(const double *partial, int job, int qblocks, int k)
+{
+    double s = 0.0;
+    const double *base = partial + (size_t)job * qblocks * kPartial + k;
+    if (qblocks <= 4) {
+        double v[4];
+#pragma unroll
+        for (int u = 0; u < 4; ++u) v[u] = base[(size_t)min(u, qblocks - 1) * kPartial];
+#pragma unroll
+        for (int u = 0; u < 4; ++u)
+            if (u < qblocks) s += v[u];
+        return s;
+    }
+    for (int q0 = 0; q0 < qblocks; q0 += 8) {
+        double v[8];
+#pragma unroll
+        for (int u = 0; u < 8; ++u) v[u] = base[(size_t)min(q0 + u, qblocks - 1) * kPartial];
+#pragma unroll
+        for (int u = 0; u < 8; ++u)
+            if (q0 + u < qblocks) s += v[u];
+    }
+    return s;
+}
+
+__device__ __forceinline__ void score_pick_pair(const double *partial, int qblocks, const int32_t *lenA, const int32_t *lenC,
+                                                const uint8_t *swap, const float *cand, const int b, const int lane,
+                                                float *Tinit, double *initSum)
+{
+    const bool sw = swap != nullptr && swap[b] != 0;
+    const float na = (float)(sw ? lenC[b] : lenA[b]);
+    const float nc = (float)(sw ? lenA[b] : lenC[b]);
+    float mean = 0.f;
+    double total = 0.0;
+    if (lane < 2 * kCand) {
+        total = partial_total(partial, b * 12 + lane, qblocks, 0);
+        mean = (float)total / ((lane & 1) ? nc : na);
+    }
+    int pick = 0;
+    float best = 0.f;
+    for (int k = 0; k < kCand; ++k) {
+        const float sc = fminf(__shfl(mean, 2 * k, kWave), __shfl(mean, 2 * k + 1, kWave));
+        if (k == 0 || sc < best) { best = sc; pick = k; }
+    }
+    if (initSum != nullptr && lane == 2 * pick) initSum[b] = total;
+    if (lane < 16) {
+        const float *t = cand + ((size_t)b * kCand + pick) * 3;
+        float v = (lane % 5 == 0) ? 1.f : 0.f;
+        if (lane == 3) v = t[0];
+        if (lane == 7) v = t[1];
+        if (lane == 11) v = t[2];
+        Tinit[(size_t)b * 16 + lane] = v;
+    }
+}
+
+__device__ __forceinline__ void select_pair(const double *partial, int qblocks, const int32_t *lenA, const int32_t *lenC,
+                                            const uint8_t *swap, const float *init, const float *M, int invertSwapped,
+                                            float *out, const PoseSource &fused, const double *initSum, const uint8_t *active,
+                                            const int b, const int n)
+{
+    float Mf[16];
+    if (M == nullptr) final_pose(fused, b, n, Mf);
+    const bool sw = swap != nullptr && swap[b] != 0;
+    const float na = (float)(sw ? lenC[b] : lenA[b]);
+    double s0 = 0.0;
+    bool reuse = false;
+    if (initSum != nullptr && (active == nullptr || active[b] != 0)) {
+        s0 = initSum[b];
+        reuse = s0 - s0 == 0.0;
+    }
+    if (!reuse) s0 = partial_total(partial, b * 2 + 0, qblocks, 0);
+#ifdef ICPFLOW_REUSE_STATS_TU
+    atomicAdd(&g_reuseStats[reuse ? 0 : (initSum != nullptr ? 1 : 2)], 1ull);
+#endif
+    const float e0 = (float)s0 / na;
+    const float e1 = (float)partial_total(partial, b * 2 + 1, qblocks, 0) / na;
+    const float *src = (e1 >= e0) ? init + (size_t)b * 16 : (M != nullptr ? M + (size_t)b * 16 : Mf);
+#ifdef ICPFLOW_REUSE_STATS_TU
+    if (e1 >= e0) atomicAdd(&g_reuseStats[3], 1ull);
+#endif
+    float P[16];
+    for (int k = 0; k < 16; ++k) P[k] = src[k];
+    if (sw && invertSwapped) {
+        const double a = P[0], bb = P[1], c = P[2], d = P[4], e = P[5], f = P[6], g = P[8], h = P[9],
+                     i = P[10];
+        const double tx = P[3], ty = P[7], tz = P[11];
+        const double c00 = e * i - f * h, c01 = c * h - bb * i, c02 = bb * f - c * e;
+        const double c10 = f * g - d * i, c11 = a * i - c * g, c12 = c * d - a * f;
+        const double c20 = d * h - e * g, c21 = bb * g - a * h, c22 = a * e - bb * d;
+        const double det = a * c00 + bb * c10 + c * c20;
+        const double r = 1.0 / det;
+        const double I00 = c00 * r, I01 = c01 * r, I02 = c02 * r;
+        const double I10 = c10 * r, I11 = c11 * r, I12 = c12 * r;
+        const double I20 = c20 * r, I21 = c21 * r, I22 = c22 * r;
+        P[0] = (float)I00; P[1] = (float)I01; P[2] = (float)I02;
+        P[4] = (float)I10; P[5] = (float)I11; P[6] = (float)I12;
+        P[8] = (float)I20; P[9] = (float)I21; P[10] = (float)I22;
+        P[3] = (float)(-(I00 * tx + I01 * ty + I02 * tz));
+        P[7] = (float)(-(I10 * tx + I11 * ty + I12 * tz));
+        P[11] = (float)(-(I20 * tx + I21 * ty + I22 * tz));
+        P[12] = P[13] = P[14] = 0.f; P[15] = 1.f;
+    }
+    float *o = out + (size_t)b * 16;
+    for (int k = 0; k < 16; ++k) o[k] = P[k];
+}
+
+}
diff --git a/icp_flow_amd/csrc/pose.hip b/icp_flow_amd/csrc/pose.hip
--- a/icp_flow_amd/csrc/pose.hip
+++ b/icp_flow_amd/csrc/pose.hip
@@ -1,32 +1,13 @@
 #include "common.hpp"
 #include "kernels.hpp"
 #include "posefuse.hpp"
+#ifdef ICPFLOW_REUSE_STATS
+#define ICPFLOW_REUSE_STATS_TU
+namespace icpflow { __device__ unsigned long long g_reuseStats[4]; }
+#endif
+#include "pairfold.hpp"
 
 namespace icpflow {
-
-__device__ __forceinline__ double partial_total(const double *partial, int job, int qblocks, int k)
-{
-    double s = 0.0;
-    const double *base = partial + (size_t)job * qblocks * kPartial + k;
-    if (qblocks <= 4) {
-        double v[4];
-#pragma unroll
-        for (int u = 0; u < 4; ++u) v[u] = base[(size_t)min(u, qblocks - 1) * kPartial];
-#pragma unroll
-        for (int u = 0; u < 4; ++u)
-            if (u < qblocks) s += v[u];
-        return s;
-    }
-    for (int q0 = 0; q0 < qblocks; q0 += 8) {
-        double v[8];
-#pragma unroll
-        for (int u = 0; u < 8; ++u) v[u] = base[(size_t)min(q0 + u, qblocks - 1) * kPartial];
-#pragma unroll
-        for (int u = 0; u < 8; ++u)
-            if (q0 + u < qblocks) s += v[u];
-    }
-    return s;
-}
 
 __global__ __launch_bounds__(kWave) void score_pick_kernel(const double *__restrict__ partial, int qblocks,
                                                            const int32_t *__restrict__ lenA,
@@ -35,31 +16,7 @@
                                                            const float *__restrict__ cand, int B,
                                                            float *__restrict__ Tinit, double *__restrict__ initSum)
 {
-    const int b = blockIdx.x, lane = threadIdx.x;
-    const bool sw = swap != nullptr && swap[b] != 0;
-    const float na = (float)(sw ? lenC[b] : lenA[b]);
-    const float nc = (float)(sw ? lenA[b] : lenC[b]);
-    float mean = 0.f;
-    double total = 0.0;
-    if (lane < 2 * kCand) {
-        total = partial_total(partial, b * 12 + lane, qblocks, 0);
-        mean = (float)total / ((lane & 1) ? nc : na);
-    }
-    int pick = 0;
-    float best = 0.f;
-    for (int k = 0; k < kCand; ++k) {
-        const float sc = fminf(__shfl(mean, 2 * k, kWave), __shfl(mean, 2 * k + 1, kWave));
-        if (k == 0 || sc < best) { best = sc; pick = k; }
-    }
-    if (initSum != nullptr && lane == 2 * pick) initSum[b] = total;
-    if (lane < 16) {
-        const float *t = cand + ((size_t)b * kCand + pick) * 3;
-        float v = (lane % 5 == 0) ? 1.f : 0.f;
-        if (lane == 3) v = t[0];
-        if (lane == 7) v = t[1];
-        if (lane == 11) v = t[2];
-        Tinit[(size_t)b * 16 + lane] = v;
-    }
+    score_pick_pair(partial, qblocks, lenA, lenC, swap, cand, (int)blockIdx.x, (int)threadIdx.x, Tinit, initSum);
 }
 
 hipError_t launch_score_pick(const double *partial, int qblocks, const int32_t *lenA,
@@ -103,9 +60,6 @@
     return hipGetLastError();
 }
 
-#ifdef ICPFLOW_REUSE_STATS
-__device__ unsigned long long g_reuseStats[4];
-#endif
 __global__ void select_kernel(const double *__restrict__ partial, int qblocks,
                               const int32_t *__restrict__ lenA, const int32_t *__restrict__ lenC,
                               const uint8_t *__restrict__ swap, const float *__restrict__ init,
@@ -120,50 +74,7 @@
         if (b == 0 && iters != nullptr) *iters = fused.ctrl->error ? -1 : n;
     }
     if (b >= B) return;
-    float Mf[16];
-    if (M == nullptr) final_pose(fused, b, n, Mf);
-    const bool sw = swap != nullptr && swap[b] != 0;
-    const float na = (float)(sw ? lenC[b] : lenA[b]);
-    double s0 = 0.0;
-    bool reuse = false;
-    if (initSum != nullptr && (active == nullptr || active[b] != 0)) {
-        s0 = initSum[b];
-        reuse = s0 - s0 == 0.0;
-    }
-    if (!reuse) s0 = partial_total(partial, b * 2 + 0, qblocks, 0);
-#ifdef ICPFLOW_REUSE_STATS
-    atomicAdd(&g_reuseStats[reuse ? 0 : (initSum != nullptr ? 1 : 2)], 1ull);
-#endif
-    const float e0 = (float)s0 / na;
-    const float e1 = (float)partial_total(partial, b * 2 + 1, qblocks, 0) / na;
-    const float *src = (e1 >= e0) ? init + (size_t)b * 16 : (M != nullptr ? M + (size_t)b * 16 : Mf);
-#ifdef ICPFLOW_REUSE_STATS
-    if (e1 >= e0) atomicAdd(&g_reuseStats[3], 1ull);
-#endif
-    float P[16];
-    for (int k = 0; k < 16; ++k) P[k] = src[k];
-    if (sw && invertSwapped) {
-        const double a = P[0], bb = P[1], c = P[2], d = P[4], e = P[5], f = P[6], g = P[8], h = P[9],
-                     i = P[10];
-        const double tx = P[3], ty = P[7], tz = P[11];
-        const double c00 = e * i - f * h, c01 = c * h - bb * i, c02 = bb * f - c * e;
-        const double c10 = f * g - d * i, c11 = a * i - c * g, c12 = c * d - a * f;
-        const double c20 = d * h - e * g, c21 = bb * g - a * h, c22 = a * e - bb * d;
-        const double det = a * c00 + bb * c10 + c * c20;
-        const double r = 1.0 / det;
-        const double I00 = c00 * r, I01 = c01 * r, I02 = c02 * r;
-        const double I10 = c10 * r, I11 = c11 * r, I12 = c12 * r;
-        const double I20 = c20 * r, I21 = c21 * r, I22 = c22 * r;
-        P[0] = (float)I00; P[1] = (float)I01; P[2] = (float)I02;
-        P[4] = (float)I10; P[5] = (float)I11; P[6] = (float)I12;
-        P[8] = (float)I20; P[9] = (float)I21; P[10] = (float)I22;
-        P[3] = (float)(-(I00 * tx + I01 * ty + I02 * tz));
-        P[7] = (float)(-(I10 * tx + I11 * ty + I12 * tz));
-        P[11] = (float)(-(I20 * tx + I21 * ty + I22 * tz));
-        P[12] = P[13] = P[14] = 0.f; P[15] = 1.f;
-    }
-    float *o = out + (size_t)b * 16;
-    for (int k = 0; k < 16; ++k) o[k] = P[k];
+    select_pair(partial, qblocks, lenA, lenC, swap, init, M, invertSwapped, out, fused, initSum, active, b, n);
 }
 
 hipError_t launch_select(const double *partial, int qblocks, const int32_t *lenA, const int32_t *lenC,
diff --git a/include/icpflow_hip.h b/include/icpflow_hip.h
--- a/include/icpflow_hip.h
+++ b/include/icpflow_hip.h
@@ -50,6 +50,8 @@
 #define ICPFLOW_OPT_NO_SCORE_PREBOUND (1u << 16)
 #define ICPFLOW_OPT_TWO_LAUNCH (1u << 17)
 #define ICPFLOW_OPT_NO_DIR_KEYS (1u << 18)
+#define ICPFLOW_OPT_NO_SCORE_ONE_LAUNCH (1u << 19)
+#define ICPFLOW_OPT_NO_SELECT_FOLD (1u << 20)
 
 typedef struct icpflow_profile icpflow_profile_t;
 
```

Result: slower. 245,300 (-39.3%).
